# meuleman/epilogos

Measured on AMD Instinct MI355X. Metric: Mbins scored/sec (S1, 18-state, 833 biosamples), higher is better.
Workload: dtype u8

## Files before the change

### epilogos_amd/_abi.py

```python
import ctypes as C
import re
from pathlib import Path

from . import build as _build

EPG_OK = 0
ERR_NAMES = {-1: "EPG_ERR_INVALID_ARG", -2: "EPG_ERR_UNSUPPORTED", -3: "EPG_ERR_HIP", -4: "EPG_ERR_WORKSPACE"}

HEADER = Path(__file__).resolve().parents[1] / "include" / "epilogos_amd.h"


class EpilogosHipError(RuntimeError):
    def __init__(self, code, msg):
        super().__init__("%s (%d): %s" % (ERR_NAMES.get(code, "EPG_ERR"), code, msg))
        self.code = code


_p = C.c_void_p
_i64 = C.c_int64
_i32 = C.c_int32
_u64 = C.c_uint64

PROTOTYPES = {
    "epg_version": (C.c_int, []),
    "epg_last_error": (C.c_char_p, []),
    "epg_device_cus": (C.c_int, []),
    "epg_bin_hist": (C.c_int, [_p, _i64, _i32, _i64, _i32, _p, _p, _p]),
    "epg_bin_hist_s2": (C.c_int, [_p, _i64, _i32, _i64, _i32, _p, _p, _p, _p]),
    "epg_bin_hist_parts": (C.c_int, [_i32, _p, _p, _p, _p, _i32, _p, _p, _p]),
    "epg_hist_s1": (C.c_int, [_p, _i64, _i32, _i64, _i32, _p, _p]),
    "epg_hist_s2": (C.c_int, [_p, _i64, _i32, _i64, _i32, _p, _p, _i64, _p]),
    "epg_hist_s2_from_binhist": (C.c_int, [_p, _i64, _i32, _p, _p]),
    "epg_hist_s2_from_binhist_pair": (C.c_int, [_p, _p, _i64, _i32, _p, _p]),
    "epg_combine_score_s1": (C.c_int, [_p, _i32, _p, _i64, _i32, _i32, _p, _p, _p, _p, _i64, _p]),
    "epg_hist_s3": (C.c_int, [_p, _i64, _i32, _i64, _i32, _p, _p, _i64, _p]),
    "epg_normalise_i64": (C.c_int, [_p, _i64, _p, _p, _i64, _p]),
    "epg_normalise_i32": (C.c_int, [_p, _i64, _p, _p, _i64, _p]),
    "epg_ws_bytes": (_i64, [_i32, _i64, _i32, _i32]),
    "epg_score_s1": (C.c_int, [_p, _i64, _i32, _i64, _i32, _p, _p, _p, _p, _i64, _p]),
    "epg_score_s1_from_binhist": (C.c_int, [_p, _i64, _i32, _i32, _p, _p, _p, _p, _i64, _p]),
    "epg_score_s1_from_binhist_table": (C.c_int, [_p, _i64, _i32, _i32, _p, _p, _p, _p, _p]),
    "epg_pair_scores_s1_from_binhist": (C.c_int, [_p, _p, _p, _p, _i64, _i32, _i32, _i32, _i32, _i32, _p, _p, _p, _p, _p, _p, _p, _p, _p]),
    "epg_pair_scores_s1_parts": (C.c_int, [_i32, _p, _p, _p, _p, _p, _i32, _i32, _i32, _i32, _i32, _p, _p, _p, _p, _p, _p, _p, _p, _p, _i32, _p]),
    "epg_score_s2": (C.c_int, [_p, _i64, _i32, _i64, _i32, _i64, _p, _p, _p, _p, _i64, _p]),
    "epg_score_s2_from_binhist": (C.c_int, [_p, _i64, _i32, _i32, _i64, _p, _p, _p, _p, _i64, _p]),
    "epg_score_s3": (C.c_int, [_p, _i64, _i32, _i64, _i32, _p, _p, _p, _p, _i64, _p]),
    "epg_pair_finish": (C.c_int, [_p, _p, _i64, _i32, _p, _p, _p]),
    "epg_pair_metrics": (C.c_int, [_p, _i64, _i32, _i32, _p, _p, _p]),
    "epg_quiescent": (C.c_int, [_p, _i32, _i64, _p, _i32, _i64, _i64, _i32, _p, _p]),
    "epg_null_hist": (C.c_int, [_p, _i32, _i64, _p, _i32, _i64, _i64, _i32, _i32, _i32, _u64, _i64, _p, _p, _p]),
    "epg_quiescent_from_binhist": (C.c_int, [_p, _p, _i64, _i32, _i32, _i32, _i32, _p, _p]),
    "epg_null_hist_from_binhist": (C.c_int, [_p, _p, _i64, _i32, _i32, _i32, _i32, _u64, _i64, _p, _p, _p]),
    "epg_null_hist_from_binhist_parts": (C.c_int, [_i32, _p, _p, _p, _i32, _i32, _i32, _i32, _u64, _p, _p, _p, _p]),
    "epg_pair_count_null_parts": (C.c_int, [_i32, _p, _p, _p, _i32, _i32, _p, _p, _i32, _p, _p, _p, _u64, _p, _p, _p, _p]),
    "epg_simsearch_ws_bytes": (_i64, [_i64, _i32, _i32, _i32]),
    "epg_simsearch": (C.c_int, [_p, _i64, _i32, _i32, _p, _i32, _p, _i32, _u64, _p, _i64, _p, _p, _p, _p]),
    "epg_simsearch_reduce": (C.c_int, [_p, _i64, _i32, _i32, _p, _p, _p]),
    "epg_simsearch_slices": (C.c_int, [_p, _i64, _i32, _i32, _i32, _p, _i32, _p, _p]),
    "epg_test_force": (C.c_int, [_i32, _i32]),
}

_lib = None


def header_symbols():
    txt = re.sub(r"/\*.*?\*/", "", HEADER.read_text(), flags=re.S)
    return sorted(set(re.findall(r"\b(epg_[a-z0-9_]+)\s*\(", txt)))


def lib_path():
    import os
    p = os.environ.get("EPILOGOS_HIP_LIB")
    return Path(p) if p else _build.LIB_PATH


def _header_abi_version():
    m = re.search(r"^#define\s+EPG_ABI_VERSION\s+(\d+)", HEADER.read_text(), flags=re.M)
    if m is None:
        raise RuntimeError("EPG_ABI_VERSION not found in %s" % HEADER)
    return int(m.group(1))


ABI_VERSION = _header_abi_version()


def load():
    global _lib
    if _lib is not None:
        return _lib
    import torch
    path = lib_path()
    if not path.exists():
        raise EpilogosHipError(-3, "%s is missing: build it with `python -m epilogos_amd.build` "
                                   "(there is no CPU fallback)" % path)
    lib = C.CDLL(str(path))
    for name, (res, args) in PROTOTYPES.items():
        fn = getattr(lib, name)
        fn.restype = res
        fn.argtypes = args
    if lib.epg_version() != ABI_VERSION:
        raise EpilogosHipError(-3, "%s has ABI version %d, this package speaks %d: rebuild it with `python -m epilogos_amd.build`"
                               % (path, lib.epg_version(), ABI_VERSION))
    _lib = lib
    return lib


def check(rc):
    if rc < 0:
        raise EpilogosHipError(rc, load().epg_last_error().decode(errors="replace"))
    return rc


def call(name, *args):
    return check(getattr(load(), name)(*args))
```

### epilogos_amd/build.py

```python
import os
import shutil
import subprocess
from pathlib import Path

PKG = Path(__file__).resolve().parent
ROOT = PKG.parent
CSRC = PKG / "csrc"
LIB_DIR = PKG / "_lib"
LIB_PATH = LIB_DIR / "libepilogos_hip.so"
SOURCES = ["epg_abi.hip", "epg_s1.hip", "epg_s2.hip", "epg_s3.hip", "epg_s3_transpose.hip", "epg_s3_gemm.hip", "epg_s3_lanes.hip", "epg_null.hip", "epg_wide.hip", "epg_simsearch.hip",
           "epg_simsearch_prep.hip"]
HEADERS = [CSRC / "epg_common.h", CSRC / "epg_count.h", ROOT / "include" / "epilogos_amd.h"]
ARCH = "gfx950"


def _hipcc():
    exe = shutil.which("hipcc") or "/opt/rocm/bin/hipcc"
    if not os.path.exists(exe):
        raise RuntimeError("hipcc not found: cannot build libepilogos_hip.so")
    return exe


def is_stale():
    if not LIB_PATH.exists():
        return True
    t = LIB_PATH.stat().st_mtime
    deps = [CSRC / s for s in SOURCES] + HEADERS
    return any(d.stat().st_mtime > t for d in deps)


IO_LIB_PATH = LIB_DIR / "libepilogos_io.so"
IO_SOURCE = CSRC / "epg_io.cpp"
IO_HEADER = ROOT / "include" / "epilogos_io.h"


def io_is_stale():
    if not IO_LIB_PATH.exists():
        return True
    t = IO_LIB_PATH.stat().st_mtime
    return any(f.stat().st_mtime > t for f in (IO_SOURCE, IO_HEADER, CSRC / "epg_deflate.h", CSRC / "epg_inflate.h", CSRC / "epg_crc32.h"))


def build_io_library(force=False, verbose=False):
    if not force and not io_is_stale():
        return IO_LIB_PATH
    LIB_DIR.mkdir(parents=True, exist_ok=True)
    cxx = shutil.which("g++") or shutil.which("c++")
    if cxx is None:
        raise RuntimeError("g++ not found: cannot build libepilogos_io.so")
    tmp = LIB_DIR / (IO_LIB_PATH.name + ".tmp.%d" % os.getpid())
    cmd = [cxx, "-O3", "-std=c++17", "-fPIC", "-shared", "-pthread", "-I" + str(ROOT / "include"), str(IO_SOURCE),
           "-lz", "-o", str(tmp)]
    if verbose:
        print(" ".join(cmd), flush=True)
    res = subprocess.run(cmd, capture_output=True, text=True)
    if res.returncode != 0:
        raise RuntimeError("g++ failed:\n" + res.stdout + res.stderr)
    os.replace(tmp, IO_LIB_PATH)
    return IO_LIB_PATH


OBJ_DIR = LIB_DIR / "obj"


def _compile_one(src, obj, extra_flags, verbose):
    cmd = [_hipcc(), "--offload-arch=" + ARCH, "-O3", "-std=c++17", "-fPIC", "-c",
           "-I" + str(ROOT / "include"), "-I" + str(CSRC), *extra_flags, str(src), "-o", str(obj)]
    if verbose:
        print(" ".join(cmd), flush=True)
    res = subprocess.run(cmd, capture_output=True, text=True)
    if res.returncode != 0:
        raise RuntimeError("hipcc failed on %s:\n%s%s" % (src.name, res.stdout, res.stderr))


def build_library(force=False, verbose=False, extra_flags=()):
    if os.environ.get("EPILOGOS_BUILD_EXPERIMENTS") == "1":
        extra_flags = tuple(extra_flags) + ("-DEPILOGOS_BUILD_EXPERIMENTS",)
    if not force and not is_stale():
        return LIB_PATH
    from concurrent.futures import ThreadPoolExecutor
    OBJ_DIR.mkdir(parents=True, exist_ok=True)
    flag_tag = OBJ_DIR / "flags.txt"
    flags_now = " ".join(extra_flags)
    same_flags = flag_tag.exists() and flag_tag.read_text() == flags_now
    hdr_t = max(h.stat().st_mtime for h in HEADERS)
    todo, objs = [], []
    for s in SOURCES:
        src, obj = CSRC / s, OBJ_DIR / (s + ".o")
        objs.append(obj)
        if force or not same_flags or not obj.exists() or obj.stat().st_mtime < max(src.stat().st_mtime, hdr_t):
            todo.append((src, obj))
    jobs = max(1, min(len(todo), int(os.environ.get("EPILOGOS_BUILD_JOBS", os.cpu_count() or 4))))
    if todo:
        with ThreadPoolExecutor(max_workers=jobs) as pool:
            for f in [pool.submit(_compile_one, src, obj, extra_flags, verbose) for src, obj in todo]:
                f.result()
        flag_tag.write_text(flags_now)
    tmp = LIB_DIR / (LIB_PATH.name + ".tmp.%d" % os.getpid())
    cmd = [_hipcc(), "--offload-arch=" + ARCH, "-fPIC", "-shared", *[str(o) for o in objs], "-o", str(tmp)]
    if verbose:
        print(" ".join(cmd), flush=True)
    res = subprocess.run(cmd, capture_output=True, text=True)
    if res.returncode != 0:
        raise RuntimeError("hipcc link failed:\n" + res.stdout + res.stderr)
    os.replace(tmp, LIB_PATH)
    return LIB_PATH


if __name__ == "__main__":
    print(build_library(force=True, verbose=True))
    print(build_io_library(force=True, verbose=True))
```

### epilogos_amd/csrc/epg_s1.hip

```cpp
#include "epg_count.h"

#include <stdlib.h>
#include <string.h>

namespace epg {

typedef unsigned short k1_v2u16 __attribute__((ext_vector_type(2)));

constexpr int K1P_LD = 17;

template <int SC, bool FULL, bool PAIRS, typename Loop>
__device__ __forceinline__ void bin_hist_body(int Sout_, u64* __restrict__ counts, int nmax, u64* __restrict__ counts2, Loop&& loop) {
    constexpr int S = SC;
    constexpr int ND = (S + 1) / 2;
    const int Sout = FULL ? S : Sout_;
    const int ROWB = 2 * Sout;
    __shared__ u64 s_cnt[S + 1];
    __shared__ __attribute__((aligned(16))) char s_stage[4][32 * 2 * S];
    constexpr int PG = (S + 2) / 3, PSP = 3 * PG, PROLES = PG * (PG + 1) / 2, PSLICE = PROLES <= 64 ? 64 / PROLES : 1;
    static_assert(!PAIRS || (FULL && PROLES <= 64), "the pair counts need a compile-time row width and at most 64 block roles");
    __shared__ u32 s_pair[PAIRS ? 4 * PSP * K1P_LD : 1];
    __shared__ u64 s_c2[PAIRS ? S * S : 1];
    const int lane = threadIdx.x & 63, wave = threadIdx.x >> 6;
    const int j = lane & 3, b = lane >> 2;
    if (threadIdx.x <= S) s_cnt[threadIdx.x] = 0;
    if (PAIRS) {
        for (int e = threadIdx.x; e < S * S; e += 256) s_c2[e] = 0;
        for (int e = threadIdx.x; e < 4 * PSP * K1P_LD; e += 256) s_pair[e] = 0;
    }
    __syncthreads();
    u16* H = nullptr;
    int pgi = -1, pgj = 0, pkq = 0;
    u64 pacc[PAIRS ? 9 : 1], prs[PAIRS ? 3 : 1];
    if (PAIRS) {
        const int role = lane < PROLES * PSLICE ? lane / PSLICE : -1;
        pkq = lane % PSLICE;
        if (role >= 0) {
            int t = role, i = 0;
            while (t >= PG - i) { t -= PG - i; ++i; }
            pgi = i; pgj = i + t;
        }
#pragma unroll
        for (int c = 0; c < 9; ++c) pacc[c] = 0;
#pragma unroll
        for (int c = 0; c < 3; ++c) prs[c] = 0;
    }
    auto pair_counts = [&](const char* stage, int rows) {
        u32* sp = s_pair + wave * PSP * K1P_LD;
        const u16* raw = reinterpret_cast<const u16*>(stage);
        __builtin_amdgcn_wave_barrier();
        for (int e = lane; e < S * 16; e += 64) {
            const int i = e >> 4, k = e & 15;
            const u32 lo = 2 * k < rows ? raw[(2 * k) * S + i] : 0u, hi = 2 * k + 1 < rows ? raw[(2 * k + 1) * S + i] : 0u;
            sp[i * K1P_LD + k] = lo | (hi << 16);
        }
        __builtin_amdgcn_wave_barrier();
        if (pgi >= 0) {
            const u32* pi = sp + 3 * pgi * K1P_LD;
            const u32* pj = sp + 3 * pgj * K1P_LD;
            u32 part[9] = {0, 0, 0, 0, 0, 0, 0, 0, 0}, ps[3] = {0, 0, 0};
            const bool diag = pgi == pgj;
            for (int k = pkq; k < 16; k += PSLICE) {
                const u32 av[3] = {pi[k], pi[K1P_LD + k], pi[2 * K1P_LD + k]};
                const u32 bv[3] = {pj[k], pj[K1P_LD + k], pj[2 * K1P_LD + k]};
#pragma unroll
                for (int t = 0; t < 3; ++t)
#pragma unroll
                    for (int u = 0; u < 3; ++u)
                        part[3 * t + u] = __builtin_amdgcn_udot2(__builtin_bit_cast(k1_v2u16, av[t]), __builtin_bit_cast(k1_v2u16, bv[u]), part[3 * t + u], false);
                if (diag) {
#pragma unroll
                    for (int t = 0; t < 3; ++t)
                        ps[t] = __builtin_amdgcn_udot2(__builtin_bit_cast(k1_v2u16, av[t]), __builtin_bit_cast(k1_v2u16, 0x00010001u), ps[t], false);
                }
            }
#pragma unroll
            for (int c = 0; c < 9; ++c) pacc[c] += part[c];
#pragma unroll
            for (int c = 0; c < 3; ++c) prs[c] += ps[c];
        }
        __builtin_amdgcn_wave_barrier();
    };

    u32 accp[ND];
#pragma unroll
    for (int m = 0; m < ND; ++m) accp[m] = 0;
    const int flush_every = 65535 / nmax > 1 ? 65535 / nmax - 1 : 1;
    int since = 0;
    auto flush = [&]() {
        if (j == 0) {
#pragma unroll
            for (int m = 0; m < ND; ++m) {
                const u32 lo = accp[m] & 0xffffu, hi = accp[m] >> 16;
                if (lo) atomicAdd(&s_cnt[2 * m], (u64)lo);
                if (hi) atomicAdd(&s_cnt[2 * m + 1], (u64)hi);
            }
        }
#pragma unroll
        for (int m = 0; m < ND; ++m) accp[m] = 0;
        since = 0;
    };

    auto enter = [&](u16* Hpart) { H = Hpart; };
    auto epilogue = [&](int half, long row, bool valid, u32 (&cnt)[S]) {
        u32 d[ND];
        pack_reduce<S>(cnt, d);
        if (counts) {
#pragma unroll
            for (int m = 0; m < ND; ++m) accp[m] += valid ? d[m] : 0u;
            if (++since >= flush_every) flush();
        }
        if (H) {
            char* srow = &s_stage[wave][(half * 16 + b) * ROWB];
            if constexpr (FULL && (S & 1) == 0) {
#pragma unroll
                for (int k = 0; k < (ND + 3) / 4; ++k) {
                    const u32 v = sel4(d[4 * k], 4 * k + 1 < ND ? d[4 * k + 1] : 0u, 4 * k + 2 < ND ? d[4 * k + 2] : 0u,
                                       4 * k + 3 < ND ? d[4 * k + 3] : 0u, j);
                    if (4 * k + j < ND) *reinterpret_cast<u32*>(srow + 4 * (4 * k + j)) = v;
                }
            } else {
#pragma unroll
                for (int k = 0; k < (S + 3) / 4; ++k) {
                    const u32 v = (j & 2) ? (2 * k + 1 < ND ? d[2 * k + 1] : 0u) : d[2 * k];
                    const u32 c = (j & 1) ? v >> 16 : v & 0xffffu;
                    if (4 * k + j < Sout) *reinterpret_cast<u16*>(srow + 2 * (4 * k + j)) = (u16)c;
                }
            }
        }
    };
    auto finish = [&](long st, long row0, int rows) {
        if (H) store_staged(s_stage[wave], reinterpret_cast<char*>(H) + row0 * ROWB, rows * ROWB, lane);
        if constexpr (PAIRS) pair_counts(s_stage[wave], rows);
    };
    loop(enter, epilogue, finish);

    if (counts) {
        flush();
        __syncthreads();
        if ((int)threadIdx.x < Sout && s_cnt[threadIdx.x]) atomicAdd(&counts[threadIdx.x], s_cnt[threadIdx.x]);
    }
    if constexpr (PAIRS) {
        if (pgi >= 0) {
            const bool diag = pgi == pgj;
#pragma unroll
            for (int t = 0; t < 3; ++t)
#pragma unroll
                for (int u = 0; u < 3; ++u) {
                    const int i = 3 * pgi + t, jj = 3 * pgj + u;
                    u64 v = pacc[3 * t + u];
                    if (diag && t == u) v -= prs[t];
                    if (i >= S || jj >= S || !v) continue;
                    atomicAdd(&s_c2[i * S + jj], v);
                    if (!diag) atomicAdd(&s_c2[jj * S + i], v);
                }
        }
        __syncthreads();
        for (int e = threadIdx.x; e < S * S; e += 256)
            if (s_c2[e]) atomicAdd(&counts2[e], s_c2[e]);
    }
}

template <int SC, int NG, bool FULL>
__global__ __launch_bounds__(256) void k_bin_hist(const char* __restrict__ X, long R, int N, long ldx, int Sout_,
                                                   u16* __restrict__ H, u64* __restrict__ counts) {
    bin_hist_body<SC, FULL, false>(Sout_, counts, N, nullptr, [&](auto&& enter, auto&& epilogue, auto&& finish) {
        enter(H);
        tile_loop<SC, NG>(X, R, N, ldx, epilogue, finish);
    });
}

template <int SC, int NG>
__global__ __launch_bounds__(256) void k_bin_hist_s2(const char* __restrict__ X, long R, int N, long ldx, u16* __restrict__ H,
                                                      u64* __restrict__ counts, u64* __restrict__ counts2) {
    bin_hist_body<SC, true, true>(SC, counts, N, counts2, [&](auto&& enter, auto&& epilogue, auto&& finish) {
        enter(H);
        tile_loop<SC, NG>(X, R, N, ldx, epilogue, finish);
    });
}

template <int SC, int NG, bool FULL>
__global__ __launch_bounds__(256) void k_bin_hist_parts(const KhParts pt, int Sout_, u64* __restrict__ counts, int nmax) {
    bin_hist_body<SC, FULL, false>(Sout_, counts, nmax, nullptr, [&](auto&& enter, auto&& epilogue, auto&& finish) {
        tile_loop_parts<SC, NG>(pt, [&](int part) { enter(pt.h[part]); }, epilogue, finish);
    });
}

__global__ __launch_bounds__(256) void k_bin_hist_safe(const char* __restrict__ X, long row_begin, long row_end, int N,
                                                        long ldx, int S, u16* __restrict__ H, u64* __restrict__ counts, int mask = 31) {
    __shared__ u32 s_h[4][128];
    const int lane = threadIdx.x & 63, wave = threadIdx.x >> 6;
    for (long row = row_begin + (long)blockIdx.x * 4 + wave; row < row_end; row += (long)gridDim.x * 4) {
        for (int s = lane; s < S; s += 64) s_h[wave][s] = 0;
        __builtin_amdgcn_wave_barrier();
        const char* rp = X + row * ldx;
        for (int n = lane; n < N; n += 64) {
            const int v = (unsigned char)rp[n] & mask;
            if (v < S) atomicAdd(&s_h[wave][v], 1u);
        }
        __builtin_amdgcn_wave_barrier();
        for (int s = lane; s < S; s += 64) {
            const u32 c = s_h[wave][s];
            if (H) H[row * S + s] = (u16)c;
            if (counts && c) atomicAdd(&counts[s], (u64)c);
        }
        __builtin_amdgcn_wave_barrier();
    }
}

__global__ void k_s1_table(const float* __restrict__ q, int N, int S, double* __restrict__ T64, float* __restrict__ T32) {
    const long e = (long)blockIdx.x * blockDim.x + threadIdx.x;
    if (e >= (long)(N + 1) * S) return;
    const int c = (int)(e / S), s = (int)(e % S);
    const double p = (double)c / (double)N;
    const double v = kl_term(p, (double)q[s]);
    T64[e] = v;
    T32[e] = (float)v;
}

template <int S, int NG, typename OT>
__global__ __launch_bounds__(256) void k_score_s1(const char* __restrict__ X, long R, int N, long ldx,
                                                   const OT* __restrict__ T, OT* __restrict__ out) {
    constexpr int ND = (S + 1) / 2;
    constexpr int ROWB = S * (int)sizeof(OT);
    __shared__ __attribute__((aligned(16))) char s_stage[4][32 * ROWB];
    const int lane = threadIdx.x & 63, wave = threadIdx.x >> 6;
    const int j = lane & 3, b = lane >> 2;
    auto epilogue = [&](int half, long row, bool valid, u32 (&cnt)[S]) {
        u32 d[ND];
        pack_reduce<S>(cnt, d);
        OT* srow = reinterpret_cast<OT*>(&s_stage[wave][(half * 16 + b) * ROWB]);
#pragma unroll
        for (int k = 0; k < (S + 3) / 4; ++k) {
            const u32 v = (j & 2) ? (2 * k + 1 < ND ? d[2 * k + 1] : 0u) : d[2 * k];
            const u32 c = (j & 1) ? v >> 16 : v & 0xffffu;
            const int s = 4 * k + j;
            if (s < S) srow[s] = (c && valid) ? T[(long)c * S + s] : (OT)0;
        }
    };
    auto finish = [&](long st, long row0, int rows) {
        store_staged_nt(s_stage[wave], reinterpret_cast<char*>(out) + row0 * ROWB, rows * ROWB, lane);
    };
    tile_loop<S, NG>(X, R, N, ldx, epilogue, finish);
}

template <typename OT, bool LDS_T>
__global__ __launch_bounds__(LDS_T ? 1024 : 256) void k_score_s1_from_hist(const u16* __restrict__ H, long total, int S,
                                                                             const OT* __restrict__ Tg, int nent, OT* __restrict__ out,
                                                                             u64* __restrict__ zero_counts, int rev) {
    extern __shared__ __attribute__((aligned(16))) char smem_t[];
    if (zero_counts && blockIdx.x == 0 && (int)threadIdx.x < S) zero_counts[threadIdx.x] = 0;
    const OT* T = Tg;
    if (LDS_T) {
        OT* Ts = reinterpret_cast<OT*>(smem_t);
        for (int e = threadIdx.x; e < nent; e += blockDim.x) Ts[e] = Tg[e];
        __syncthreads();
        T = Ts;
    }
    const u32 cmax = (u32)(nent / S - 1);
    const long nquads = total >> 2;
    const long stride = (long)gridDim.x * blockDim.x;
    long qd = (long)blockIdx.x * blockDim.x + threadIdx.x;
    const long qtop = nquads - 1, qsgn = rev ? -1 : 1, qoff = rev ? qtop : 0;
    for (; qd + 3 * stride < nquads; qd += 4 * stride) {
        uint2 h[4];
#pragma unroll
        for (int u = 0; u < 4; ++u) h[u] = *reinterpret_cast<const uint2*>(H + 4 * (qoff + qsgn * (qd + u * stride)));
#pragma unroll
        for (int u = 0; u < 4; ++u) {
            const long e0 = 4 * (qoff + qsgn * (qd + u * stride));
            int s = (int)(e0 % S);
            const u32 c[4] = {h[u].x & 0xffffu, h[u].x >> 16, h[u].y & 0xffffu, h[u].y >> 16};
            OT v[4];
#pragma unroll
            for (int k = 0; k < 4; ++k) {
                v[k] = c[k] - 1u < cmax ? T[(long)c[k] * S + s] : (OT)0;
                s = s + 1 == S ? 0 : s + 1;
            }
            if constexpr (sizeof(OT) == 4) {
                typedef float v4f_nt __attribute__((ext_vector_type(4)));
                const v4f_nt vv = {(float)v[0], (float)v[1], (float)v[2], (float)v[3]};
                __builtin_nontemporal_store(vv, reinterpret_cast<v4f_nt*>(out + e0));
            } else {
                typedef double v2d_nt __attribute__((ext_vector_type(2)));
                const v2d_nt lo = {(double)v[0], (double)v[1]}, hi = {(double)v[2], (double)v[3]};
                __builtin_nontemporal_store(lo, reinterpret_cast<v2d_nt*>(out + e0));
                __builtin_nontemporal_store(hi, reinterpret_cast<v2d_nt*>(out + e0 + 2));
            }
        }
    }
    for (; qd < nquads; qd += stride) {
        const long e0 = 4 * (qoff + qsgn * qd);
        int s = (int)(e0 % S);
        for (int k = 0; k < 4; ++k) {
            const u32 c = H[e0 + k];
            out[e0 + k] = c - 1u < cmax ? T[(long)c * S + s] : (OT)0;
            s = s + 1 == S ? 0 : s + 1;
        }
    }
    if (blockIdx.x == 0 && threadIdx.x < (total & 3)) {
        const long e = (nquads << 2) + threadIdx.x;
        const u32 c = H[e];
        out[e] = c - 1u < cmax ? T[(long)c * S + (int)(e % S)] : (OT)0;
    }
}

template <typename IT>
__global__ __launch_bounds__(256) void k_sum_int(const IT* __restrict__ C, long n, long long* __restrict__ total) {
    long long acc = 0;
    for (long i = (long)blockIdx.x * blockDim.x + threadIdx.x; i < n; i += (long)gridDim.x * blockDim.x) acc += (long long)C[i];
    for (int off = 32; off > 0; off >>= 1) acc += __shfl_down(acc, off);
    __shared__ long long s_part[4];
    if ((threadIdx.x & 63) == 0) s_part[threadIdx.x >> 6] = acc;
    __syncthreads();
    if (threadIdx.x == 0) {
        const long long t = s_part[0] + s_part[1] + s_part[2] + s_part[3];
        if (t) atomicAdd(reinterpret_cast<u64*>(total), (u64)t);
    }
}

template <typename IT>
__global__ __launch_bounds__(256) void k_normalise(const IT* __restrict__ C, long n, const long long* __restrict__ total,
                                                    float* __restrict__ q) {
    const double tot = (double)(*total);
    for (long i = (long)blockIdx.x * blockDim.x + threadIdx.x; i < n; i += (long)gridDim.x * blockDim.x)
        q[i] = (float)((double)C[i] / tot);
}

template <typename IT>
__global__ __launch_bounds__(256) void k_normalise_small(const IT* __restrict__ C, int n, float* __restrict__ q) {
    __shared__ long long s_part[4];
    long long acc = 0;
    for (int i = threadIdx.x; i < n; i += 256) acc += (long long)C[i];
    for (int off = 32; off > 0; off >>= 1) acc += __shfl_down(acc, off);
    if ((threadIdx.x & 63) == 0) s_part[threadIdx.x >> 6] = acc;
    __syncthreads();
    const double tot = (double)(s_part[0] + s_part[1] + s_part[2] + s_part[3]);
    for (int i = threadIdx.x; i < n; i += 256) q[i] = (float)((double)C[i] / tot);
}

static int blocks_per_cu() { return g_force[FORCE_K1_BLOCKS_PER_CU] > 0 ? g_force[FORCE_K1_BLOCKS_PER_CU] : 2; }
static int grid_for_tiles(long R) {
    const long nsuper = (R + 31) >> 5;
    long blocks = (nsuper + 3) / 4;
    const long cap = (long)num_cus() * blocks_per_cu();
    if (blocks > cap) {
        const long iters = (nsuper + cap * 4 - 1) / (cap * 4);
        blocks = (nsuper + iters * 4 - 1) / (iters * 4);
    }
    if (blocks < 1) blocks = 1;
    return (int)blocks;
}

template <typename F>
static void with_count_core(int S, int ng, F&& f) {
    if (S == 15 || S == 18 || S == 25)
        with_constant<25, 15, 18>(S, [&](auto sc) {
            with_constant<0, 1, 2, 3, 4, 5, 6, 7, 8>(ng, [&](auto NG) { f(sc, NG, std::true_type{}); });
        });
    else
        with_constant<31, 15, 18, 25>(S < 15 ? 15 : S < 18 ? 18 : S < 25 ? 25 : 31,
                                      [&](auto sc) { f(sc, std::integral_constant<int, 0>{}, std::false_type{}); });
}

static long fast_rows(long R, int N, long ldx) {
    const long chunks = (N + 15) / 16;
    const long over = 16 * chunks - ldx;
    if (over <= 0) return R;
    const long unsafe = (over + ldx - 1) / ldx;
    return R > unsafe ? R - unsafe : 0;
}

extern "C" int epg_bin_hist(const int8_t* X8, int64_t R, int32_t N, int64_t ldx, int32_t S, uint16_t* H, int64_t* counts, void* stream) {
    hipStream_t st = (hipStream_t)stream;
    if (R < 0 || N < 1 || ldx < N || S < 1) return fail(EPG_ERR_INVALID_ARG, "bin_hist: bad shape R=%lld N=%d ldx=%lld S=%d", (long long)R, N, (long long)ldx, S);
    if (S > 127) return fail(EPG_ERR_UNSUPPORTED, "bin_hist: S=%d > 127 (states are int8)", S);
    if (N > 65535) return fail(EPG_ERR_UNSUPPORTED, "bin_hist: N=%d > 65535 (uint16 per-bin counts)", N);
    if (R == 0) return EPG_OK;
    if (!X8) return fail(EPG_ERR_INVALID_ARG, "bin_hist: X is NULL");
    if (H && (reinterpret_cast<uintptr_t>(H) & 15)) return fail(EPG_ERR_INVALID_ARG, "bin_hist: H must be 16-byte aligned");
    const char* X = reinterpret_cast<const char*>(X8);
    u64* cnt = reinterpret_cast<u64*>(counts);
    if (S > 31) {
        hipLaunchKernelGGL(k_bin_hist_safe, dim3((unsigned)((R + 3) / 4 < num_cus() * 32L ? (R + 3) / 4 : num_cus() * 32L)), dim3(256), 0, st, X, 0L,
                           (long)R, N, ldx, S, H, cnt, 255);
        EPG_LAUNCH_CHECK("k_bin_hist_safe");
        return EPG_OK;
    }
    const long Rf = fast_rows(R, N, ldx);
    if (Rf > 0) {
        with_count_core(S, (N + 127) / 128, [&](auto SC, auto NG, auto MODEL) {
            hipLaunchKernelGGL((k_bin_hist<SC, NG, MODEL && (SC & 1) == 0>), dim3(grid_for_tiles(Rf)), dim3(256), 0, st, X, Rf, N, ldx, S, H, cnt);
        });
        EPG_LAUNCH_CHECK("k_bin_hist");
    }
    if (Rf < R) {
        hipLaunchKernelGGL(k_bin_hist_safe, dim3((unsigned)((R - Rf + 3) / 4 < 1024 ? (R - Rf + 3) / 4 : 1024)), dim3(256), 0, st, X, Rf, (long)R, N, ldx, S, H, cnt);
        EPG_LAUNCH_CHECK("k_bin_hist_safe");
    }
    return EPG_OK;
}

extern "C" int epg_bin_hist_s2(const int8_t* X8, int64_t R, int32_t N, int64_t ldx, int32_t S, uint16_t* H, int64_t* counts, int64_t* counts2,
                               void* stream) {
    hipStream_t st = (hipStream_t)stream;
    if (!H || !counts2) return fail(EPG_ERR_INVALID_ARG, "bin_hist_s2: H and counts2 are required");
    const bool fused = (S == 15 || S == 18 || S == 25) && R > 0 && N >= 1 && N <= 1024 && ldx >= N && X8 &&
                       !(reinterpret_cast<uintptr_t>(H) & 15) && fast_rows(R, N, ldx) == R;
    if (!fused) {
        int rc = epg_bin_hist(X8, R, N, ldx, S, H, counts, stream);
        if (rc) return rc;
        return epg_hist_s2_from_binhist(H, R, S, counts2, stream);
    }
    const char* X = reinterpret_cast<const char*>(X8);
    u64* c1 = reinterpret_cast<u64*>(counts);
    u64* c2 = reinterpret_cast<u64*>(counts2);
    with_constant<25, 18, 15>(S, [&](auto SC) {
        with_constant<8, 1, 2, 3, 4, 5, 6, 7>((N + 127) / 128, [&](auto NG) {
            hipLaunchKernelGGL((k_bin_hist_s2<decltype(SC)::value, NG>), dim3(grid_for_tiles(R)), dim3(256), 0, st, X, R, N, ldx, H, c1, c2);
        });
    });
    EPG_LAUNCH_CHECK("k_bin_hist_s2");
    return EPG_OK;
}

extern "C" int epg_bin_hist_parts(int32_t nparts, const int8_t* const* X, const int64_t* R, const int32_t* N, const int64_t* ldx, int32_t S,
                                  uint16_t* const* H, int64_t* counts, void* stream) {
    hipStream_t st = (hipStream_t)stream;
    if (nparts < 0 || (nparts && (!X || !R || !N || !ldx))) return fail(EPG_ERR_INVALID_ARG, "bin_hist_parts: NULL argument array");
    if (S < 1 || S > 127) return fail(EPG_ERR_UNSUPPORTED, "bin_hist_parts: S=%d outside 1..127", S);
    for (int p = 0; p < nparts; ++p) {
        if (R[p] < 0 || (R[p] && (N[p] < 1 || ldx[p] < N[p]))) return fail(EPG_ERR_INVALID_ARG, "bin_hist_parts: bad shape of part %d", p);
        if (R[p] && N[p] > 65535) return fail(EPG_ERR_UNSUPPORTED, "bin_hist_parts: N=%d > 65535 (uint16 per-bin counts)", N[p]);
        if (R[p] && !X[p]) return fail(EPG_ERR_INVALID_ARG, "bin_hist_parts: X of part %d is NULL", p);
        if (H && H[p] && (reinterpret_cast<uintptr_t>(H[p]) & 15)) return fail(EPG_ERR_INVALID_ARG, "bin_hist_parts: H of part %d must be 16-byte aligned", p);
    }
    if (S > 31) {
        for (int p = 0; p < nparts; ++p) {
            const int rc = epg_bin_hist(X[p], R[p], N[p], ldx[p], S, H ? H[p] : nullptr, counts, stream);
            if (rc) return rc;
        }
        return EPG_OK;
    }
    u64* cnt = reinterpret_cast<u64*>(counts);
    auto cls = [](int n) { const int ng = (n + 127) / 128; return ng <= 8 ? ng : 0; };
    bool seen[9] = {false, false, false, false, false, false, false, false, false};
    for (int p = 0; p < nparts; ++p)
        if (R[p]) seen[cls(N[p])] = true;
    for (int c = 0; c <= 8; ++c) {
        if (!seen[c]) continue;
        for (int p0 = 0; p0 < nparts;) {
            KhParts pt;
            memset(&pt, 0, sizeof(pt));
            long supers = 0;
            int nmax = 1, p = p0;
            for (; p < nparts && pt.n < KH_MAXP; ++p) {
                if (!R[p] || cls(N[p]) != c) continue;
                const long Rf = fast_rows(R[p], N[p], ldx[p]);
                if (Rf < R[p]) {
                    hipLaunchKernelGGL(k_bin_hist_safe, dim3((unsigned)((R[p] - Rf + 3) / 4 < 1024 ? (R[p] - Rf + 3) / 4 : 1024)), dim3(256), 0, st,
                                       reinterpret_cast<const char*>(X[p]), Rf, (long)R[p], N[p], (long)ldx[p], S, H ? H[p] : nullptr, cnt);
                    EPG_LAUNCH_CHECK("k_bin_hist_safe");
                }
                if (Rf == 0) continue;
                const int k = pt.n++;
                pt.x[k] = reinterpret_cast<const char*>(X[p]);
                pt.h[k] = H ? H[p] : nullptr;
                pt.rows[k] = Rf;
                pt.ldx[k] = ldx[p];
                pt.n_cols[k] = N[p];
                pt.st0[k] = supers;
                supers += (Rf + 31) / 32;
                if (N[p] > nmax) nmax = N[p];
            }
            pt.st0[pt.n] = supers;
            p0 = p;
            if (pt.n == 0) break;
            with_count_core(S, c, [&](auto SC, auto NG, auto) {
                hipLaunchKernelGGL((k_bin_hist_parts<SC, NG, (NG > 0 && (SC & 1) == 0)>), dim3(grid_for_tiles(supers * 32)), dim3(256), 0, st, pt, S,
                                   cnt, nmax);
            });
            EPG_LAUNCH_CHECK("k_bin_hist_parts");
        }
    }
    return EPG_OK;
}

static int64_t s1_table_bytes(int N, int S) { return align_up((int64_t)(N + 1) * S * 8, 256) + align_up((int64_t)(N + 1) * S * 4, 256); }

int64_t s1_ws_bytes(int64_t R, int N, int S) {
    return s1_table_bytes(N, S) + 256 + align_up(R * S * 2, 256);
}

static int build_s1_table(const float* q, int N, int S, void* ws, double** T64, float** T32, hipStream_t st) {
    *T64 = reinterpret_cast<double*>(ws);
    *T32 = reinterpret_cast<float*>(reinterpret_cast<char*>(ws) + align_up((int64_t)(N + 1) * S * 8, 256));
    const long n = (long)(N + 1) * S;
    hipLaunchKernelGGL(k_s1_table, dim3((int)((n + 255) / 256)), dim3(256), 0, st, q, N, S, *T64, *T32);
    EPG_LAUNCH_CHECK("k_s1_table");
    return EPG_OK;
}
static int check_score_from_hist_args(const uint16_t* H, const double* out64, const float* out32) {
    if ((reinterpret_cast<uintptr_t>(H) & 7) != 0) return fail(EPG_ERR_INVALID_ARG, "score_s1_from_binhist: H must be 8-byte aligned");
    if ((out32 && (reinterpret_cast<uintptr_t>(out32) & 15)) || (out64 && (reinterpret_cast<uintptr_t>(out64) & 15)))
        return fail(EPG_ERR_INVALID_ARG, "score_s1_from_binhist: outputs must be 16-byte aligned");
    return EPG_OK;
}

template <typename OT>
static int launch_score_s1_from_hist_t(const uint16_t* H, long total, int32_t S, const OT* T, int nent, OT* out, u64* zero_counts, hipStream_t st) {
    const size_t tbytes = (size_t)nent * sizeof(OT);
    const int rev = 1;
    if (tbytes <= 150 * 1024) {
        const int per_cu = tbytes <= 75 * 1024 ? 2 : 1;
        long nb = (total / 4 + 4095) / 4096;
        if (nb > (long)num_cus() * per_cu) nb = (long)num_cus() * per_cu;
        if (nb < 1) nb = 1;
        auto kern = k_score_s1_from_hist<OT, true>;
        static DynLds lds_attr;
        EPG_HIP(ensure_dyn_lds(lds_attr, reinterpret_cast<const void*>(kern), 150 * 1024));
        hipLaunchKernelGGL(kern, dim3((int)nb), dim3(1024), tbytes, st, H, total, S, T, nent, out, zero_counts, rev);
    } else {
        long nb = (total / 4 + 1023) / 1024;
        if (nb > num_cus() * 8L) nb = num_cus() * 8L;
        if (nb < 1) nb = 1;
        hipLaunchKernelGGL((k_score_s1_from_hist<OT, false>), dim3((int)nb), dim3(256), 0, st, H, total, S, T, nent, out, zero_counts, rev);
    }
    EPG_LAUNCH_CHECK("k_score_s1_from_hist");
    return EPG_OK;
}

static int launch_score_s1_from_hist(const uint16_t* H, int64_t R, int32_t N, int32_t S, const double* T64, const float* T32,
                                     double* out64, float* out32, hipStream_t st, u64* zero_counts = nullptr) {
    const long total = (long)R * S;
    const int nent = (N + 1) * S;
    int rc = EPG_OK;
    if (out32) rc = launch_score_s1_from_hist_t<float>(H, total, S, T32, nent, out32, zero_counts, st);
    if (!rc && out64) rc = launch_score_s1_from_hist_t<double>(H, total, S, T64, nent, out64, out32 ? nullptr : zero_counts, st);
    return rc;
}


extern "C" int epg_score_s1_from_binhist(const uint16_t* H, int64_t R, int32_t N, int32_t S, const float* q, double* out64, float* out32,
                                         void* ws, int64_t ws_bytes, void* stream) {
    hipStream_t st = (hipStream_t)stream;
    if (R < 0 || N < 1 || S < 1) return fail(EPG_ERR_INVALID_ARG, "score_s1: bad shape");
    if (R == 0) return EPG_OK;
    if (!H || !q || !ws) return fail(EPG_ERR_INVALID_ARG, "score_s1_from_binhist: NULL argument");
    if (ws_bytes < s1_table_bytes(N, S)) return fail(EPG_ERR_WORKSPACE, "score_s1: workspace %lld < %lld bytes", (long long)ws_bytes, (long long)s1_table_bytes(N, S));
    int rc = check_score_from_hist_args(H, out64, out32);
    if (rc) return rc;
    double* T64; float* T32;
    rc = build_s1_table(q, N, S, ws, &T64, &T32, st);
    if (rc) return rc;
    return launch_score_s1_from_hist(H, R, N, S, T64, T32, out64, out32, st);
}

extern "C" int epg_score_s1_from_binhist_table(const uint16_t* H, int64_t R, int32_t N, int32_t S, const double* T64, const float* T32,
                                               double* out64, float* out32, void* stream) {
    if (R < 0 || N < 1 || S < 1) return fail(EPG_ERR_INVALID_ARG, "score_s1: bad shape");
    if (R == 0) return EPG_OK;
    if (!H || (out64 && !T64) || (out32 && !T32)) return fail(EPG_ERR_INVALID_ARG, "score_s1_from_binhist_table: NULL argument");
    if ((T64 && (reinterpret_cast<uintptr_t>(T64) & 7)) || (T32 && (reinterpret_cast<uintptr_t>(T32) & 3)))
        return fail(EPG_ERR_INVALID_ARG, "score_s1_from_binhist_table: misaligned table");
    int rc = check_score_from_hist_args(H, out64, out32);
    if (rc) return rc;
    return launch_score_s1_from_hist(H, R, N, S, T64, T32, out64, out32, (hipStream_t)stream);
}

__global__ __launch_bounds__(256) void k_s1_combine(const u64* __restrict__ counts, int N, int S, float* __restrict__ q,
                                                     double* __restrict__ T64, float* __restrict__ T32) {
    __shared__ long long s_c[128];
    __shared__ double s_q[128];
    const int t = threadIdx.x;
    if (t < S) s_c[t] = (long long)counts[t];
    __syncthreads();
    if (t < S) {
        long long tot = 0;
        for (int s = 0; s < S; ++s) tot += s_c[s];
        const float qf = (float)((double)s_c[t] / (double)tot);
        if (blockIdx.x == 0) q[t] = qf;
        s_q[t] = (double)qf;
    }
    __syncthreads();
    const int e = blockIdx.x * 256 + t;
    if (e < (N + 1) * S) {
        const int c = e / S, s = e - c * S;
        const double v = kl_term((double)c / (double)N, s_q[s]);
        T64[e] = v;
        T32[e] = (float)v;
    }
}

extern "C" int epg_combine_score_s1(int64_t* counts, int32_t rezero, const uint16_t* H, int64_t R, int32_t N, int32_t S, float* q,
                                    double* out64, float* out32, void* ws, int64_t ws_bytes, void* stream) {
    hipStream_t st = (hipStream_t)stream;
    if (R < 0 || N < 1 || S < 1) return fail(EPG_ERR_INVALID_ARG, "combine_score_s1: bad shape R=%lld N=%d S=%d", (long long)R, N, S);
    if (S > 127) return fail(EPG_ERR_UNSUPPORTED, "combine_score_s1: S=%d > 127 (states are int8)", S);
    if (!counts || !q || !ws || (R > 0 && !H)) return fail(EPG_ERR_INVALID_ARG, "combine_score_s1: NULL argument");
    if (ws_bytes < s1_table_bytes(N, S)) return fail(EPG_ERR_WORKSPACE, "combine_score_s1: workspace %lld < %lld bytes", (long long)ws_bytes, (long long)s1_table_bytes(N, S));
    int rc = check_score_from_hist_args(H, out64, out32);
    if (rc) return rc;
    double* T64 = reinterpret_cast<double*>(ws);
    float* T32 = reinterpret_cast<float*>(reinterpret_cast<char*>(ws) + align_up((int64_t)(N + 1) * S * 8, 256));
    const long nent = (long)(N + 1) * S;
    hipLaunchKernelGGL(k_s1_combine, dim3((unsigned)((nent + 255) / 256)), dim3(256), 0, st, reinterpret_cast<const u64*>(counts), N, S, q, T64, T32);
    EPG_LAUNCH_CHECK("k_s1_combine");
    if (R == 0 || (!out32 && !out64)) {
        if (rezero) EPG_HIP(hipMemsetAsync(counts, 0, (size_t)S * 8, st));
        return EPG_OK;
    }
    return launch_score_s1_from_hist(H, R, N, S, T64, T32, out64, out32, st, rezero ? reinterpret_cast<u64*>(counts) : nullptr);
}

extern "C" int epg_hist_s1(const int8_t* X, int64_t R, int32_t N, int64_t ldx, int32_t S, int64_t* counts, void* stream) {
    if (!counts) return fail(EPG_ERR_INVALID_ARG, "hist_s1: counts is NULL");
    return epg_bin_hist(X, R, N, ldx, S, nullptr, counts, stream);
}

extern "C" int epg_score_s1(const int8_t* X8, int64_t R, int32_t N, int64_t ldx, int32_t S, const float* q, double* out64, float* out32,
                            void* ws, int64_t ws_bytes, void* stream) {
    hipStream_t st = (hipStream_t)stream;
    if (R < 0 || N < 1 || ldx < N || S < 1) return fail(EPG_ERR_INVALID_ARG, "score_s1: bad shape");
    if (S > 127) return fail(EPG_ERR_UNSUPPORTED, "score_s1: S=%d > 127 (states are int8)", S);
    if (R == 0) return EPG_OK;
    if (!X8 || !q || !ws) return fail(EPG_ERR_INVALID_ARG, "score_s1: NULL argument");
    if ((out32 && (reinterpret_cast<uintptr_t>(out32) & 15)) || (out64 && (reinterpret_cast<uintptr_t>(out64) & 15)))
        return fail(EPG_ERR_INVALID_ARG, "score_s1: outputs must be 16-byte aligned");
    const long Rf = fast_rows(R, N, ldx);
    const bool fused = S == 18 && Rf == R;
    if (!fused) {
        if (ws_bytes < s1_ws_bytes(R, N, S)) return fail(EPG_ERR_WORKSPACE, "score_s1: workspace %lld < %lld bytes", (long long)ws_bytes, (long long)s1_ws_bytes(R, N, S));
        u16* H = reinterpret_cast<u16*>(reinterpret_cast<char*>(ws) + s1_table_bytes(N, S));
        int rc = epg_bin_hist(X8, R, N, ldx, S, H, nullptr, stream);
        if (rc) return rc;
        return epg_score_s1_from_binhist(H, R, N, S, q, out64, out32, ws, s1_table_bytes(N, S), stream);
    }
    if (ws_bytes < s1_table_bytes(N, S)) return fail(EPG_ERR_WORKSPACE, "score_s1: workspace %lld < %lld bytes", (long long)ws_bytes, (long long)s1_table_bytes(N, S));
    double* T64; float* T32;
    int rc = build_s1_table(q, N, S, ws, &T64, &T32, st);
    if (rc) return rc;
    const char* X = reinterpret_cast<const char*>(X8);
    with_constant<0, 1, 2, 3, 4, 5, 6, 7, 8>((N + 127) / 128, [&](auto NG) {
        if (out32) hipLaunchKernelGGL((k_score_s1<18, NG, float>), dim3(grid_for_tiles(R)), dim3(256), 0, st, X, R, N, ldx, T32, out32);
        if (out64) hipLaunchKernelGGL((k_score_s1<18, NG, double>), dim3(grid_for_tiles(R)), dim3(256), 0, st, X, R, N, ldx, T64, out64);
    });
    EPG_LAUNCH_CHECK("k_score_s1");
    return EPG_OK;
}

template <typename IT>
static int normalise_impl(const IT* C, int64_t n, float* q, void* ws, int64_t ws_bytes, hipStream_t st) {
    if (n < 1 || !C || !q || !ws) return fail(EPG_ERR_INVALID_ARG, "normalise: bad argument");
    if (ws_bytes < 8) return fail(EPG_ERR_WORKSPACE, "normalise: workspace needs 8 bytes");
    if (n <= 4096) {
        hipLaunchKernelGGL((k_normalise_small<IT>), dim3(1), dim3(256), 0, st, C, (int)n, q);
        EPG_LAUNCH_CHECK("k_normalise_small");
        return EPG_OK;
    }
    long long* total = reinterpret_cast<long long*>(ws);
    EPG_HIP(hipMemsetAsync(total, 0, 8, st));
    long blocks = (n + 255) / 256;
    if (blocks > num_cus() * 8L) blocks = num_cus() * 8L;
    hipLaunchKernelGGL((k_sum_int<IT>), dim3((int)blocks), dim3(256), 0, st, C, (long)n, total);
    hipLaunchKernelGGL((k_normalise<IT>), dim3((int)blocks), dim3(256), 0, st, C, (long)n, total, q);
    EPG_LAUNCH_CHECK("k_normalise");
    return EPG_OK;
}

extern "C" int epg_normalise_i64(const int64_t* C, int64_t n, float* q, void* ws, int64_t ws_bytes, void* stream) {
    return normalise_impl<long long>(reinterpret_cast<const long long*>(C), n, q, ws, ws_bytes, (hipStream_t)stream);
}
extern "C" int epg_normalise_i32(const int32_t* C, int64_t n, float* q, void* ws, int64_t ws_bytes, void* stream) {
    return normalise_impl<int>(C, n, q, ws, ws_bytes, (hipStream_t)stream);
}

}
```

### epilogos_amd/engine.py

```python
import ctypes as C

import numpy as np
import torch

from . import _abi
from ._abi import EpilogosHipError

ROW_ALIGN = 16


def require_gpu():
    if not torch.cuda.is_available():
        raise EpilogosHipError(-3, "no HIP device visible to torch: the epilogos_amd engine has no CPU fallback")
    _abi.load()


def _ptr(t):
    return C.c_void_p(t.data_ptr()) if t is not None else None


def _stream():
    return C.c_void_p(torch.cuda.current_stream().cuda_stream)


def padded_width(N):
    return (N + ROW_ALIGN - 1) // ROW_ALIGN * ROW_ALIGN


def alloc_states(R, N, device="cuda"):
    return torch.empty((R, padded_width(N)), dtype=torch.int8, device=device)


PLACE_MIN_BYTES = 1 << 30
PLACE_BLOCK = 4 << 30
PLACE_SEARCH_AT = 2
PLACE_TRIES = 8
PLACE_BUDGET_MS = 50.0
PLACE_DEEP_AT = 4
PLACE_DEEP_TRIES = 24
PLACE_DEEP_WALL_MS = 5000.0
PLACE_GAP = 0.03
PLACE_SURE = 1.10
PLACE_WIN = 0.01
_placement = {}


def _storage_users(t):
    f = getattr(torch._C, "_storage_Use_Count", None)
    if f is None:
        return None
    return int(f(t.untyped_storage()._cdata)) - 1


def _probe_slices(R, rows=1 << 20):
    m = min(rows, R // 3) // 32 * 32
    if m <= 0:
        return [(0, R)]
    return [(0, m), ((R - m) // 2 // 32 * 32, (R - m) // 2 // 32 * 32 + m), ((R - m) // 32 * 32, (R - m) // 32 * 32 + m)]


def _probe_ms(X, N, S, Hflat, counts, slices, reps=2):
    ev = [torch.cuda.Event(enable_timing=True) for _ in range(2)]
    H = None if Hflat is None else Hflat[:X.shape[0] * S * 2].view(torch.int16).view(X.shape[0], S)
    for k in range(reps + 1):
        if k == 1:
            ev[0].record()
        for lo, hi in slices:
            bin_hist(X[lo:hi], N, S, counts=counts, H=None if H is None else H[lo:hi], want_hist=H is not None)
    ev[1].record()
    ev[1].synchronize()
    return ev[0].elapsed_time(ev[1]) / reps


def place_decide(ratios, excluded=(), gap=PLACE_GAP, sure=PLACE_SURE):
    live = [i for i in range(len(ratios)) if i not in set(excluded)]
    if not live:
        return None, "none"
    order = sorted(live, key=lambda i: ratios[i])
    best = order[0]
    if ratios[best] <= sure:
        return best, "sure"
    allo = sorted(range(len(ratios)), key=lambda i: ratios[i])
    steps = [(ratios[allo[k + 1]] / ratios[allo[k]] - 1.0, k) for k in range(len(allo) - 1)]
    if steps:
        step, k = max(steps)
        if step >= gap:
            lower = [i for i in allo[:k + 1] if i not in set(excluded)]
            if lower:
                return lower[0], "two-levels"
    return best, "one-level"


def placement_enabled():
    import os
    if os.environ.get("EPILOGOS_PLACEMENT", "1") == "0" or getattr(torch._C, "_storage_Use_Count", None) is None:
        return False
    try:
        lws = int(os.environ.get("LOCAL_WORLD_SIZE", "1"))
    except ValueError:
        lws = 1
    return lws <= max(torch.cuda.device_count(), 1)


def _order_after_last_user(st):
    prev, cur = st.get("stream"), torch.cuda.current_stream()
    if prev is not None and prev != cur:
        ev = torch.cuda.Event()
        ev.record(prev)
        cur.wait_event(ev)
    st["stream"] = cur


def alloc_hist(X, N, S):
    import os
    R = X.shape[0]
    dev = X.device
    hbytes = R * S * 2
    plain = lambda: torch.empty((R, S), dtype=torch.int16, device=dev)
    if X.numel() < PLACE_MIN_BYTES or not placement_enabled():
        return plain()
    st = _placement.get(dev.index)
    stor = X.untyped_storage()
    key = (stor.data_ptr(), stor.nbytes())
    view = lambda home: home[:hbytes].view(torch.int16).view(R, S)
    eager = os.environ.get("EPILOGOS_PLACEMENT_EAGER") == "1"
    if st is not None and st["home"] is not None and st["home"].numel() >= hbytes:
        users = _storage_users(st["home"])
        if users is None or users > 1:
            st["report"]["plain_while_home_in_use"] = st["report"].get("plain_while_home_in_use", 0) + 1
            return plain()
        if st["key"] == key:
            st["report"]["reuses"] = st["report"].get("reuses", 0) + 1
            _order_after_last_user(st)
            return view(st["home"])
        counts = zeros_counts(S, device=dev)
        slices = _probe_slices(R)
        r = _probe_ms(X, N, S, st["home"], counts, slices) / _probe_ms(X, N, S, None, counts, slices)
        if r <= PLACE_SURE:
            st["key"] = key
            st["report"].update(revalidated=st["report"].get("revalidated", 0) + 1, ratio=round(r, 3))
            _order_after_last_user(st)
            return view(st["home"])
        st = None
        _placement.pop(dev.index, None)
    if st is None or st["key"] != key:
        st = _placement[dev.index] = {"key": key, "home": None, "report": {"jobs_seen": 0, "tier": "none yet"}, "stream": None, "seen": 0, "tier": 0}
    st["seen"] += 1
    st["report"]["jobs_seen"] = st["seen"]
    want = 0
    if st["tier"] < 1 and (eager or st["seen"] >= PLACE_SEARCH_AT):
        want = 1
    elif st["tier"] == 1 and (eager or st["seen"] >= PLACE_DEEP_AT):
        want = 2
    if not want:
        return plain()
    deep = want == 2
    home, h_plain, report = _place_search(X, N, S, int(os.environ.get("EPILOGOS_PLACEMENT_TRIES", PLACE_DEEP_TRIES if deep else PLACE_TRIES)),
                                          3 * PLACE_BUDGET_MS if deep else PLACE_BUDGET_MS, PLACE_DEEP_WALL_MS if deep else 10 * PLACE_BUDGET_MS,
                                          stop_at_slow_alloc=not deep)
    report.update(tier="deep" if deep else "quick", jobs_seen=st["seen"], reuses=0)
    if deep and "quick" not in report:
        report["quick"] = {k: st["report"].get(k) for k in ("decision", "ratios", "blocks_tried", "search_ms")}
    if home is None and report["picked"] == 0 and report["decision"].startswith("plain allocation kept (sure"):
        want = 2
    st.update(home=home, report=report, stream=torch.cuda.current_stream(), tier=want)
    if home is None and eager and want == 1:
        return alloc_hist(X, N, S)
    return view(home) if home is not None else h_plain


PLACE_SLOW_ALLOC_MS = 20.0


def _place_search(X, N, S, tries, budget_ms, wall_ms, stop_at_slow_alloc=False):
    import time
    R = X.shape[0]
    dev = X.device
    hbytes = R * S * 2
    t_start = time.perf_counter()
    counts = zeros_counts(S, device=dev)
    slices = _probe_slices(R)
    whole = [(0, R)]
    spent = [0.0]

    def probe(cand, where, reps=2):
        ms = _probe_ms(X, N, S, cand, counts, where, reps=reps)
        spent[0] += ms * (reps + 1)
        return ms

    base = probe(None, slices)
    block = max(PLACE_BLOCK, (hbytes + 4095) // 4096 * 4096)
    h_plain = torch.empty((R, S), dtype=torch.int16, device=dev)
    cands, ratios = [h_plain.view(torch.int8).view(-1)], []
    t0 = probe(cands[0], slices)
    base = min(base, probe(None, slices))
    ratios.append(t0 / base)
    whole_ms, excluded, alloc_ms = {}, [], []

    def walk_on():
        k = len(cands) - 1
        if k >= tries or spent[0] >= budget_ms or (time.perf_counter() - t_start) * 1e3 >= wall_ms:
            return False
        if stop_at_slow_alloc and alloc_ms and alloc_ms[-1] > PLACE_SLOW_ALLOC_MS:
            return False
        free, _total = torch.cuda.mem_get_info(dev)
        if free < block + 16 * hbytes + (8 << 30):
            return False
        t0 = time.perf_counter()
        try:
            cands.append(torch.empty(block, dtype=torch.int8, device=dev))
        except RuntimeError:
            return False
        torch.cuda.synchronize(dev)
        alloc_ms.append((time.perf_counter() - t0) * 1e3)
        ratios.append(probe(cands[-1], slices) / base)
        return True

    pick, verdict = place_decide(ratios, excluded)
    while True:
        while verdict not in ("sure", "two-levels") and walk_on():
            pick, verdict = place_decide(ratios, excluded)
        if pick in (None, 0):
            break
        if slices == whole:
            whole_ms = {0: ratios[0] * base, pick: ratios[pick] * base}
        else:
            if 0 not in whole_ms:
                whole_ms[0] = probe(cands[0], whole, reps=1)
            whole_ms[pick] = probe(cands[pick], whole, reps=1)
        if whole_ms[pick] < whole_ms[0] * (1.0 - PLACE_WIN):
            break
        excluded.append(pick)
        if len(excluded) >= 3 or spent[0] >= 2 * budget_ms:
            pick = 0
            break
        pick, verdict = place_decide(ratios, excluded)
        verdict += " (after %d pick(s) that lost over the whole matrix)" % len(excluded)
    if pick is None or pick in excluded:
        pick = 0
    good = pick != 0
    report = {"probe": "k_bin_hist over 3 x %d bins of the matrix: with the H store into a candidate / counts only; candidate 0 is the plain "
                       "allocation, the others heads of %d GiB blocks allocated one after the other" % (slices[0][1] - slices[0][0], block >> 30),
              "decision": verdict if good else "plain allocation kept (%s)" % verdict, "good": good, "picked": pick, "ratio": round(ratios[pick], 3),
              "ratios": [round(r, 3) for r in ratios], "whole_matrix_ms": {str(i): round(v, 4) for i, v in whole_ms.items()},
              "lost_over_the_whole_matrix": excluded, "blocks_tried": len(cands) - 1,
              "walked_GiB": round(sum(c.numel() for c in cands[1:]) / 2**30, 1),
              "block_alloc_ms": [round(a, 1) for a in alloc_ms],
              "rules": {"sure_at_or_under": PLACE_SURE, "two_levels_apart_by": PLACE_GAP, "must_beat_plain_by": PLACE_WIN,
                        "max_blocks": tries, "max_probe_ms": budget_ms, "max_wall_ms": wall_ms},
              "ms_counts_only": round(base, 4), "probe_device_ms": round(spent[0], 2),
              "left_in_torch_cache_GiB": round(sum(c.numel() for i, c in enumerate(cands) if i and i != pick) / 2**30, 1)}
    home = cands[pick] if good else None
    del cands
    report["search_ms"] = round((time.perf_counter() - t_start) * 1e3, 2)
    return home, h_plain, report


def placement_report(device=None):
    idx = torch.cuda.current_device() if device is None else torch.device(device).index
    st = _placement.get(idx)
    return None if st is None else dict(st["report"])


def release_placement():
    _placement.clear()


def states_to_device(x, device="cuda"):
    x = np.ascontiguousarray(x)
    R, N = x.shape
    ldx = padded_width(N)
    host = np.full((R, ldx), -1, dtype=np.int8)
    host[:, :N] = x.astype(np.int8)
    return torch.from_numpy(host).to(device)


def _check_states(X, N):
    if X.dtype != torch.int8 or X.dim() != 2 or not X.is_cuda or X.stride(1) != 1:
        raise ValueError("state matrix must be a 2-D int8 CUDA tensor with unit column stride")
    if N > X.shape[1]:
        raise ValueError("N exceeds the row width")
    return X.shape[0], X.stride(0)


def zeros_counts(n, dtype=torch.int64, device="cuda"):
    return torch.zeros(n, dtype=dtype, device=device)


def bin_hist(X, N, S, want_hist=True, counts=None, want_counts=True, H=None):
    R, ldx = _check_states(X, N)
    if H is None and want_hist:
        H = torch.empty((R, S), dtype=torch.int16, device=X.device)
    if want_counts and counts is None:
        counts = zeros_counts(S, device=X.device)
    _abi.call("epg_bin_hist", _ptr(X), R, N, ldx, S, _ptr(H), _ptr(counts) if want_counts else None, _stream())
    return H, counts


def bin_hist_s2(X, N, S, counts2=None, H=None, counts=None):
    R, ldx = _check_states(X, N)
    if H is None:
        H = torch.empty((R, S), dtype=torch.int16, device=X.device)
    if counts2 is None:
        counts2 = zeros_counts(S * S, device=X.device)
    _abi.call("epg_bin_hist_s2", _ptr(X), R, N, ldx, S, _ptr(H), _ptr(counts), _ptr(counts2), _stream())
    return H, counts2


def _ptr_array(ts):
    return (C.c_void_p * len(ts))(*[t.data_ptr() if t is not None and t.numel() else None for t in ts])


def hist_rows_flat(rows, S, device, dtype=torch.int16):
    starts, at = [], 0
    for r in rows:
        starts.append(at)
        at += (r + 7) // 8 * 8
    return torch.empty((max(at, 1), S), dtype=dtype, device=device), starts


def hist_rows_alloc(rows, S, device):
    flat, starts = hist_rows_flat(rows, S, device)
    return [flat[a:a + r] for a, r in zip(starts, rows)]


def bin_hist_parts(Xs, Ns, S, counts=None, want_hist=True, Hs=None):
    n = len(Xs)
    if n == 0:
        return [], counts
    shapes = [_check_states(X, N) if X.shape[0] else (0, max(N, 1)) for X, N in zip(Xs, Ns)]
    dev = Xs[0].device
    if Hs is None and want_hist:
        Hs = hist_rows_alloc([r for r, _l in shapes], S, dev)
    _abi.call("epg_bin_hist_parts", n, _ptr_array(Xs), (C.c_int64 * n)(*[r for r, _l in shapes]), (C.c_int32 * n)(*[int(N or 1) for N in Ns]),
              (C.c_int64 * n)(*[l for _r, l in shapes]), S, _ptr_array(Hs) if Hs is not None else None, _ptr(counts), _stream())
    return Hs, counts


def null_hist_from_binhist_parts(HAs, HBs, n_cols, S, ga, gb, seed, row0s, stream=None):
    n = len(HAs)
    if n == 0:
        return [], []
    rows = [h.shape[0] for h in HAs]
    dev = HAs[0].device
    OAs, OBs = hist_rows_alloc(rows, S, dev), hist_rows_alloc(rows, S, dev)
    _abi.call("epg_null_hist_from_binhist_parts", n, _ptr_array(HAs), _ptr_array(HBs), (C.c_int64 * n)(*rows), S, n_cols, ga, gb, seed,
              (C.c_int64 * n)(*[int(r) for r in row0s]), _ptr_array(OAs), _ptr_array(OBs),
              _stream() if stream is None else C.c_void_p(stream.cuda_stream))
    return OAs, OBs


def pair_count_null_parts(XAs, XBs, NA, NB, S, seed, row0s, counts=None):
    n = len(XAs)
    sa = [_check_states(X, NA) if X.shape[0] else (0, padded_width(NA)) for X in XAs]
    sb = [_check_states(X, NB) if X.shape[0] else (0, padded_width(NB)) for X in XBs]
    rows = [r for r, _l in sa]
    if rows != [r for r, _l in sb]:
        raise ValueError("paired inputs must have the same number of bins")
    dev = XAs[0].device
    H = hist_rows_alloc(rows + rows, S, dev)
    O = hist_rows_alloc(rows + rows, S, dev)
    _abi.call("epg_pair_count_null_parts", n, _ptr_array(XAs), _ptr_array(XBs), (C.c_int64 * n)(*rows), NA, NB,
              (C.c_int64 * n)(*[l for _r, l in sa]), (C.c_int64 * n)(*[l for _r, l in sb]), S, _ptr_array(H[:n]), _ptr_array(H[n:]),
              _ptr(counts), seed, (C.c_int64 * n)(*[int(r) for r in row0s]), _ptr_array(O[:n]), _ptr_array(O[n:]), _stream())
    return H[:n], H[n:], O[:n], O[n:]


def hist_s2_from_binhist(H, S, counts=None):
    if counts is None:
        counts = zeros_counts(S * S, device=H.device)
    _abi.call("epg_hist_s2_from_binhist", _ptr(H), H.shape[0], S, _ptr(counts), _stream())
    return counts


def hist_s2_from_binhist_pair(HA, HB, S, counts=None):
    if HA.shape != HB.shape:
        raise ValueError("paired histograms must have the same shape")
    if counts is None:
        counts = zeros_counts(S * S, device=HA.device)
    _abi.call("epg_hist_s2_from_binhist_pair", _ptr(HA), _ptr(HB), HA.shape[0], S, _ptr(counts), _stream())
    return counts


def hist_s3_ws_bytes(R, N, S):
    return max(int(_abi.call("epg_ws_bytes", 3, R, N, S)), 256)


def hist_s3(X, N, S, counts=None, use_workspace=True, ws=None):
    R, ldx = _check_states(X, N)
    if counts is None:
        counts = zeros_counts(N * N * S * S, dtype=torch.int32, device=X.device)
    if use_workspace:
        if ws is None:
            ws = torch.empty(hist_s3_ws_bytes(R, N, S), dtype=torch.uint8, device=X.device)
        _abi.call("epg_hist_s3", _ptr(X), R, N, ldx, S, _ptr(counts), _ptr(ws), ws.numel(), _stream())
    else:
        _abi.call("epg_hist_s3", _ptr(X), R, N, ldx, S, _ptr(counts), None, 0, _stream())
    return counts


def normalise(counts, q=None, ws=None):
    if q is None:
        q = torch.empty(counts.numel(), dtype=torch.float32, device=counts.device)
    if ws is None:
        ws = torch.empty(256, dtype=torch.uint8, device=counts.device)
    name = {torch.int64: "epg_normalise_i64", torch.int32: "epg_normalise_i32"}[counts.dtype]
    _abi.call(name, _ptr(counts), counts.numel(), _ptr(q), _ptr(ws), ws.numel(), _stream())
    return q


def _outs(R, S, device, want32, want64, out32=None, out64=None):
    o32 = out32 if out32 is not None else (torch.empty((R, S), dtype=torch.float32, device=device) if want32 else None)
    o64 = out64 if out64 is not None else (torch.empty((R, S), dtype=torch.float64, device=device) if want64 else None)
    return o32, o64


def workspace(saliency, R, N, S, device="cuda"):
    return _ws(saliency, R, N, S, device)


def _ws(saliency, R, N, S, device):
    nbytes = _abi.call("epg_ws_bytes", saliency, R, N, S)
    return torch.empty(max(nbytes, 256), dtype=torch.uint8, device=device)


def score_s1(X, N, S, q, want32=True, want64=False, out32=None, out64=None, ws=None):
    R, ldx = _check_states(X, N)
    o32, o64 = _outs(R, S, X.device, want32, want64, out32, out64)
    if ws is None:
        ws = _ws(1, R, N, S, X.device)
    _abi.call("epg_score_s1", _ptr(X), R, N, ldx, S, _ptr(q), _ptr(o64), _ptr(o32), _ptr(ws), ws.numel(), _stream())
    return o32, o64


def score_s1_from_binhist(H, N, S, q, want32=True, want64=False, out32=None, out64=None, ws=None):
    R = H.shape[0]
    o32, o64 = _outs(R, S, H.device, want32, want64, out32, out64)
    if ws is None:
        ws = _ws(1, 0, N, S, H.device)
    _abi.call("epg_score_s1_from_binhist", _ptr(H), R, N, S, _ptr(q), _ptr(o64), _ptr(o32), _ptr(ws), ws.numel(),
              _stream())
    return o32, o64


def score_s1_from_binhist_table(H, N, S, T64=None, T32=None, out32=None, out64=None):
    R = H.shape[0]
    for T, dt in ((T64, torch.float64), (T32, torch.float32)):
        if T is not None and (T.dtype != dt or T.numel() != (N + 1) * S or not T.is_contiguous()):
            raise ValueError("S1 table must be a contiguous [N + 1, S] tensor of its output's dtype")
    o32, o64 = _outs(R, S, H.device, T32 is not None, T64 is not None, out32, out64)
    _abi.call("epg_score_s1_from_binhist_table", _ptr(H), R, N, S, _ptr(T64), _ptr(T32), _ptr(o64), _ptr(o32), _stream())
    return o32, o64


def combine_score_s1(counts, H, N, S, q=None, want32=True, want64=False, out32=None, out64=None, ws=None, rezero=False):
    R = H.shape[0]
    o32, o64 = _outs(R, S, H.device, want32, want64, out32, out64)
    if q is None:
        q = torch.empty(S, dtype=torch.float32, device=H.device)
    if ws is None:
        ws = _ws(1, 0, N, S, H.device)
    _abi.call("epg_combine_score_s1", _ptr(counts), 1 if rezero else 0, _ptr(H), R, N, S, _ptr(q), _ptr(o64), _ptr(o32),
              _ptr(ws), ws.numel(), _stream())
    return q, o32, o64


def s1_tables(counts, N, S, q=None, ws=None):
    dev = counts.device
    if q is None:
        q = torch.empty(S, dtype=torch.float32, device=dev)
    if ws is None:
        ws = _ws(1, 0, N, S, dev)
    _abi.call("epg_combine_score_s1", _ptr(counts), 0, None, 0, N, S, _ptr(q), None, None, _ptr(ws), ws.numel(), _stream())
    nent = (N + 1) * S
    off = (nent * 8 + 255) // 256 * 256
    return q, ws[:nent * 8].view(torch.float64), ws[off:off + nent * 4].view(torch.float32)


def score_s2(X, N, S, q, perms=None, want32=True, want64=False):
    R, ldx = _check_states(X, N)
    perms = N * (N - 1) if perms is None else perms
    o32, o64 = _outs(R, S, X.device, want32, want64)
    ws = _ws(2, R, N, S, X.device)
    _abi.call("epg_score_s2", _ptr(X), R, N, ldx, S, perms, _ptr(q), _ptr(o64), _ptr(o32), _ptr(ws), ws.numel(),
              _stream())
    return o32, o64


def score_s2_from_binhist(H, N, S, q, perms=None, want32=True, want64=False, out32=None, out64=None, ws=None):
    R = H.shape[0]
    perms = N * (N - 1) if perms is None else perms
    o32, o64 = _outs(R, S, H.device, want32, want64, out32, out64)
    if ws is None:
        ws = _ws(2, 0, N, S, H.device)
    _abi.call("epg_score_s2_from_binhist", _ptr(H), R, N, S, perms, _ptr(q), _ptr(o64), _ptr(o32), _ptr(ws),
              ws.numel(), _stream())
    return o32, o64


def score_s3(X, N, S, q, want32=True, want64=False, ws=None):
    R, ldx = _check_states(X, N)
    o32, o64 = _outs(R, S, X.device, want32, want64)
    if ws is None:
        ws = _ws(3, R, N, S, X.device)
    _abi.call("epg_score_s3", _ptr(X), R, N, ldx, S, _ptr(q), _ptr(o64), _ptr(o32), _ptr(ws), ws.numel(), _stream())
    return o32, o64


def pair_scores_s1_from_binhist(HA, HB, HnA, HnB, S, NA, NB, ga, gb, TA, TB, TnA, TnB):
    R = HA.shape[0]
    dev = HA.device
    delta = torch.empty((R, S), dtype=torch.float32, device=dev)
    null = torch.empty(R, dtype=torch.float32, device=dev)
    dist = torch.empty(R, dtype=torch.float32, device=dev)
    maxdiff = torch.empty(R, dtype=torch.int32, device=dev)
    _abi.call("epg_pair_scores_s1_from_binhist", _ptr(HA), _ptr(HB), _ptr(HnA), _ptr(HnB), R, S, NA, NB, ga, gb, _ptr(TA), _ptr(TB), _ptr(TnA),
              _ptr(TnB), _ptr(delta), _ptr(null), _ptr(dist), _ptr(maxdiff), _stream())
    return delta, null, dist, maxdiff


def pair_scores_s1_parts(parts, S, NA, NB, ga, gb, TA, TB, TnA, TnB, qstate=None):
    n = len(parts)
    if n == 0:
        return []
    dev = parts[0][0].device
    outs = []
    for HA, _HB, _HnA, _HnB in parts:
        R = HA.shape[0]
        outs.append({"delta": torch.empty((R, S), dtype=torch.float32, device=dev), "null": torch.empty(R, dtype=torch.float32, device=dev),
                     "rdist": torch.empty(R, dtype=torch.float32, device=dev), "mdiff": torch.empty(R, dtype=torch.int32, device=dev),
                     "quies": torch.empty(R, dtype=torch.uint8, device=dev) if qstate is not None else None})
    arr = lambda ts: (C.c_void_p * n)(*[t.data_ptr() if t is not None and t.numel() else None for t in ts])
    rows = (C.c_int64 * n)(*[p[0].shape[0] for p in parts])
    _abi.call("epg_pair_scores_s1_parts", n, arr([p[0] for p in parts]), arr([p[1] for p in parts]), arr([p[2] for p in parts]),
              arr([p[3] for p in parts]), rows, S, NA, NB, ga, gb, _ptr(TA), _ptr(TB), _ptr(TnA), _ptr(TnB), arr([o["delta"] for o in outs]),
              arr([o["null"] for o in outs]), arr([o["rdist"] for o in outs]), arr([o["mdiff"] for o in outs]),
              arr([o["quies"] for o in outs]) if qstate is not None else None, -1 if qstate is None else int(qstate), _stream())
    return outs


def pair_finish(a, b, want_dist=True):
    R, S = a.shape
    delta = torch.empty_like(a)
    dist = torch.empty(R, dtype=torch.float32, device=a.device) if want_dist else None
    _abi.call("epg_pair_finish", _ptr(a), _ptr(b), R, S, _ptr(delta), _ptr(dist), _stream())
    return delta, dist


def pair_metrics(delta, roundtrip=True):
    R, S = delta.shape
    dist = torch.empty(R, dtype=torch.float32, device=delta.device)
    maxdiff = torch.empty(R, dtype=torch.int32, device=delta.device)
    _abi.call("epg_pair_metrics", _ptr(delta), R, S, 1 if roundtrip else 0, _ptr(dist), _ptr(maxdiff), _stream())
    return dist, maxdiff


def quiescent(XA, NA, XB, NB, qstate):
    R, ldxa = _check_states(XA, NA)
    R2, ldxb = _check_states(XB, NB)
    if R != R2:
        raise ValueError("paired inputs must have the same number of bins")
    mask = torch.empty(R, dtype=torch.uint8, device=XA.device)
    _abi.call("epg_quiescent", _ptr(XA), NA, ldxa, _ptr(XB), NB, ldxb, R, qstate, _ptr(mask), _stream())
    return mask


def null_hist(XA, NA, XB, NB, S, ga, gb, seed, row0=0):
    R, ldxa = _check_states(XA, NA)
    _, ldxb = _check_states(XB, NB)
    HA = torch.empty((R, S), dtype=torch.int16, device=XA.device)
    HB = torch.empty((R, S), dtype=torch.int16, device=XA.device)
    _abi.call("epg_null_hist", _ptr(XA), NA, ldxa, _ptr(XB), NB, ldxb, R, S, ga, gb, seed, row0, _ptr(HA), _ptr(HB),
              _stream())
    return HA, HB


_hip_rt = None


def _pinned_bytes(nbytes):
    global _hip_rt
    if _hip_rt is None:
        for name in ("libamdhip64.so", "libamdhip64.so.7", "libamdhip64.so.6"):
            try:
                _hip_rt = C.CDLL(name)
                break
            except OSError:
                continue
        if _hip_rt is None:
            _hip_rt = False
    if _hip_rt:
        import weakref
        ptr = C.c_void_p()
        if _hip_rt.hipHostMalloc(C.byref(ptr), C.c_size_t(int(nbytes)), C.c_uint(0)) == 0 and ptr.value:
            base = (C.c_int8 * int(nbytes)).from_address(ptr.value)
            weakref.finalize(base, _hip_rt.hipHostFree, C.c_void_p(ptr.value))
            t = torch.from_numpy(np.frombuffer(base, dtype=np.int8))
            if t.is_pinned():
                return t
            del t
    return torch.empty(int(nbytes), dtype=torch.int8, pin_memory=True)


class PinnedPool:

    def __init__(self, n_buffers=3, in_order=True):
        import threading
        self.cv = threading.Condition()
        self.free = [None] * n_buffers
        self.next = 0
        self.in_order = in_order
        self.aborted = False
        self.weights = {}
        self.target = 0
        self.waiting = set()
        self.closed = False

    def hint(self, weights):
        self.weights = dict(weights)

    def abort(self):
        with self.cv:
            self.aborted = True
            self.cv.notify_all()

    def acquire(self, ticket, nbytes):
        import os, sys, time
        trace = os.environ.get("EPILOGOS_TIMING") == "2"
        t_in = time.perf_counter()
        with self.cv:
            self.waiting.add(ticket)
            first = lambda: not self.weights or self.weights.get(ticket, 0) >= max(self.weights.get(t, 0) for t in self.waiting)
            self.cv.wait_for(lambda: self.aborted or ((not self.in_order or self.next == ticket) and len(self.free) > 0 and first()))
            self.waiting.discard(ticket)
            if self.aborted:
                raise RuntimeError("staging pool aborted")
            buf = self.free.pop()
            self.next += 1
            self.cv.notify_all()
        w = self.weights.get(ticket)
        if w and nbytes:
            self.target = max(self.target, int(nbytes / w * max(self.weights.values()) * 1.05))
        t_got = time.perf_counter()
        grew = 0
        if buf is None or buf.numel() < nbytes:
            buf = None
            buf = _pinned_bytes(max(int(nbytes), self.target, 1 << 20))
            grew = buf.numel()
        if trace:
            print("    [pool] ticket %2d: waited %.2f s for a staging buffer%s  (at %.3f)" % (
                ticket, t_got - t_in, ", page-locked %.2f GB in %.2f s" % (grew / 1e9, time.perf_counter() - t_got) if grew else "",
                time.perf_counter()), file=sys.stderr, flush=True)
        return buf

    def skip(self, ticket):
        if not self.in_order:
            return
        with self.cv:
            self.cv.wait_for(lambda: self.aborted or self.next >= ticket)
            if self.next == ticket:
                self.next += 1
            self.cv.notify_all()

    def release(self, buf):
        with self.cv:
            if self.closed:
                return
            self.free.append(buf)
            self.cv.notify_all()

    def close(self, background=True):
        import threading
        with self.cv:
            self.closed = True
            bufs, self.free = [b for b in self.free if b is not None], []
        if not bufs:
            return

        def work(bufs=bufs):
            while bufs:
                bufs.pop()
        if background:
            threading.Thread(target=work, name="epilogos-staging-close", daemon=True).start()
        else:
            work()


def upload_states(pinned, R, ldx, copy_stream, device="cuda"):
    with torch.cuda.stream(copy_stream):
        X = torch.empty((R, ldx), dtype=torch.int8, device=device)
        if R:
            X.copy_(pinned[:R * ldx].view(R, ldx), non_blocking=True)
        ev = torch.cuda.Event()
        ev.record(copy_stream)
    X.record_stream(torch.cuda.current_stream())
    return X, ev


def quiescent_from_binhist(HA, NA, HB, NB, S, qstate):
    R = HA.shape[0]
    mask = torch.empty(R, dtype=torch.uint8, device=HA.device)
    _abi.call("epg_quiescent_from_binhist", _ptr(HA), _ptr(HB), R, S, NA, NB, qstate, _ptr(mask), _stream())
    return mask


def null_hist_from_binhist(HA, HB, n_cols, S, ga, gb, seed, row0=0, stream=None):
    if HA.shape != HB.shape:
        raise ValueError("paired histograms must have the same shape")
    OA, OB = torch.empty_like(HA), torch.empty_like(HB)
    _abi.call("epg_null_hist_from_binhist", _ptr(HA), _ptr(HB), HA.shape[0], S, n_cols, ga, gb, seed, row0, _ptr(OA), _ptr(OB),
              _stream() if stream is None else C.c_void_p(stream.cuda_stream))
    return OA, OB


def hist_to_numpy(H):
    return H.cpu().numpy().view(np.uint16)
```

Baseline: 5804.

## Pack per-bin S1 histograms as three 10-bit counts per 32-bit word

Adds a packed histogram layout that stores three 10-bit state counts in each uint32 instead of one uint16 per state. It provides packed variants of bin_hist, bin_hist_parts, the table-based S1 scoring and combine_score_s1, including a new scoring kernel that decodes the packed words. The aim is to cut the histogram's memory footprint and the bytes moved between counting and scoring. It only applies when S is a multiple of 3 up to 30 and N is at most 1023, and the engine picks the packed path only when the histogram tensor is int32, so whether the default pipeline uses it is not shown.

```diff
diff --git a/epilogos_amd/_abi.py b/epilogos_amd/_abi.py
--- a/epilogos_amd/_abi.py
+++ b/epilogos_amd/_abi.py
@@ -60,7 +60,20 @@
     "epg_test_force": (C.c_int, [_i32, _i32]),
 }
 
+PRIVATE_HEADER = Path(__file__).resolve().parent / "csrc" / "epg_packed.h"
+PRIVATE_PROTOTYPES = {
+    "epgs_bin_hist_packed": (C.c_int, [_p, _i64, _i32, _i64, _i32, _p, _p, _p]),
+    "epgs_bin_hist_parts_packed": (C.c_int, [_i32, _p, _p, _p, _p, _i32, _p, _p, _p]),
+    "epgs_score_s1_from_packed_table": (C.c_int, [_p, _i64, _i32, _i32, _p, _p, _p, _p, _p]),
+    "epgs_combine_score_s1_packed": (C.c_int, [_p, _i32, _p, _i64, _i32, _i32, _p, _p, _p, _p, _i64, _p]),
+}
+
 _lib = None
+
+
+def private_header_symbols():
+    txt = re.sub(r"/\*.*?\*/", "", PRIVATE_HEADER.read_text(), flags=re.S)
+    return sorted(set(re.findall(r"\b(epgs_[a-z0-9_]+)\s*\(", txt)))
 
 
 def header_symbols():
@@ -94,7 +107,7 @@
         raise EpilogosHipError(-3, "%s is missing: build it with `python -m epilogos_amd.build` "
                                    "(there is no CPU fallback)" % path)
     lib = C.CDLL(str(path))
-    for name, (res, args) in PROTOTYPES.items():
+    for name, (res, args) in list(PROTOTYPES.items()) + list(PRIVATE_PROTOTYPES.items()):
         fn = getattr(lib, name)
         fn.restype = res
         fn.argtypes = args
diff --git a/epilogos_amd/build.py b/epilogos_amd/build.py
--- a/epilogos_amd/build.py
+++ b/epilogos_amd/build.py
@@ -10,7 +10,7 @@
 LIB_PATH = LIB_DIR / "libepilogos_hip.so"
 SOURCES = ["epg_abi.hip", "epg_s1.hip", "epg_s2.hip", "epg_s3.hip", "epg_s3_transpose.hip", "epg_s3_gemm.hip", "epg_s3_lanes.hip", "epg_null.hip", "epg_wide.hip", "epg_simsearch.hip",
            "epg_simsearch_prep.hip"]
-HEADERS = [CSRC / "epg_common.h", CSRC / "epg_count.h", ROOT / "include" / "epilogos_amd.h"]
+HEADERS = [CSRC / "epg_common.h", CSRC / "epg_count.h", CSRC / "epg_packed.h", ROOT / "include" / "epilogos_amd.h"]
 ARCH = "gfx950"
 
 
diff --git a/epilogos_amd/csrc/epg_packed.h b/epilogos_amd/csrc/epg_packed.h
--- /dev/null
+++ b/epilogos_amd/csrc/epg_packed.h
@@ -0,0 +1,21 @@
+#pragma once
+#include <stdint.h>
+
+#ifdef __cplusplus
+extern "C" {
+#endif
+
+int epgs_bin_hist_packed(const int8_t* X, int64_t R, int32_t N, int64_t ldx, int32_t S, uint32_t* P, int64_t* counts, void* stream);
+
+int epgs_bin_hist_parts_packed(int32_t nparts, const int8_t* const* X, const int64_t* R, const int32_t* N, const int64_t* ldx, int32_t S,
+                               uint32_t* const* P, int64_t* counts, void* stream);
+
+int epgs_score_s1_from_packed_table(const uint32_t* P, int64_t R, int32_t N, int32_t S, const double* T64, const float* T32, double* out64,
+                                    float* out32, void* stream);
+
+int epgs_combine_score_s1_packed(int64_t* counts, int32_t rezero, const uint32_t* P, int64_t R, int32_t N, int32_t S, float* q, double* out64,
+                                 float* out32, void* ws, int64_t ws_bytes, void* stream);
+
+#ifdef __cplusplus
+}
+#endif
diff --git a/epilogos_amd/csrc/epg_s1.hip b/epilogos_amd/csrc/epg_s1.hip
--- a/epilogos_amd/csrc/epg_s1.hip
+++ b/epilogos_amd/csrc/epg_s1.hip
@@ -1,4 +1,5 @@
 #include "epg_count.h"
+#include "epg_packed.h"
 
 #include <stdlib.h>
 #include <string.h>
@@ -9,12 +10,15 @@
 
 constexpr int K1P_LD = 17;
 
-template <int SC, bool FULL, bool PAIRS, typename Loop>
+template <int SC, bool FULL, bool PAIRS, bool PACK = false, typename Loop>
 __device__ __forceinline__ void bin_hist_body(int Sout_, u64* __restrict__ counts, int nmax, u64* __restrict__ counts2, Loop&& loop) {
     constexpr int S = SC;
     constexpr int ND = (S + 1) / 2;
+    constexpr int PWC = (S + 2) / 3;
+    static_assert(!(PACK && PAIRS), "the pair counts read uint16 rows");
     const int Sout = FULL ? S : Sout_;
-    const int ROWB = 2 * Sout;
+    const int PW = FULL ? PWC : (Sout + 2) / 3;
+    const int ROWB = PACK ? 4 * PW : 2 * Sout;
     __shared__ u64 s_cnt[S + 1];
     __shared__ __attribute__((aligned(16))) char s_stage[4][32 * 2 * S];
     constexpr int PG = (S + 2) / 3, PSP = 3 * PG, PROLES = PG * (PG + 1) / 2, PSLICE = PROLES <= 64 ? 64 / PROLES : 1;
@@ -112,7 +116,15 @@
         }
         if (H) {
             char* srow = &s_stage[wave][(half * 16 + b) * ROWB];
-            if constexpr (FULL && (S & 1) == 0) {
+            if constexpr (PACK) {
+                auto c = [&](int s) { return s < S && (FULL || s < Sout) ? (d[s >> 1] >> (16 * (s & 1))) & 0xffffu : 0u; };
+                auto p = [&](int k) { return k < PWC ? c(3 * k) | (c(3 * k + 1) << 10) | (c(3 * k + 2) << 20) : 0u; };
+#pragma unroll
+                for (int k = 0; k < (PWC + 3) / 4; ++k) {
+                    const u32 v = sel4(p(4 * k), p(4 * k + 1), p(4 * k + 2), p(4 * k + 3), j);
+                    if (4 * k + j < PW) *reinterpret_cast<u32*>(srow + 4 * (4 * k + j)) = v;
+                }
+            } else if constexpr (FULL && (S & 1) == 0) {
 #pragma unroll
                 for (int k = 0; k < (ND + 3) / 4; ++k) {
                     const u32 v = sel4(d[4 * k], 4 * k + 1 < ND ? d[4 * k + 1] : 0u, 4 * k + 2 < ND ? d[4 * k + 2] : 0u,
@@ -161,10 +173,10 @@
     }
 }
 
-template <int SC, int NG, bool FULL>
+template <int SC, int NG, bool FULL, bool PACK = false>
 __global__ __launch_bounds__(256) void k_bin_hist(const char* __restrict__ X, long R, int N, long ldx, int Sout_,
                                                    u16* __restrict__ H, u64* __restrict__ counts) {
-    bin_hist_body<SC, FULL, false>(Sout_, counts, N, nullptr, [&](auto&& enter, auto&& epilogue, auto&& finish) {
+    bin_hist_body<SC, FULL, false, PACK>(Sout_, counts, N, nullptr, [&](auto&& enter, auto&& epilogue, auto&& finish) {
         enter(H);
         tile_loop<SC, NG>(X, R, N, ldx, epilogue, finish);
     });
@@ -179,15 +191,16 @@
     });
 }
 
-template <int SC, int NG, bool FULL>
+template <int SC, int NG, bool FULL, bool PACK = false>
 __global__ __launch_bounds__(256) void k_bin_hist_parts(const KhParts pt, int Sout_, u64* __restrict__ counts, int nmax) {
-    bin_hist_body<SC, FULL, false>(Sout_, counts, nmax, nullptr, [&](auto&& enter, auto&& epilogue, auto&& finish) {
+    bin_hist_body<SC, FULL, false, PACK>(Sout_, counts, nmax, nullptr, [&](auto&& enter, auto&& epilogue, auto&& finish) {
         tile_loop_parts<SC, NG>(pt, [&](int part) { enter(pt.h[part]); }, epilogue, finish);
     });
 }
 
 __global__ __launch_bounds__(256) void k_bin_hist_safe(const char* __restrict__ X, long row_begin, long row_end, int N,
-                                                        long ldx, int S, u16* __restrict__ H, u64* __restrict__ counts, int mask = 31) {
+                                                        long ldx, int S, u16* __restrict__ H, u64* __restrict__ counts, int mask = 31,
+                                                        int pack = 0) {
     __shared__ u32 s_h[4][128];
     const int lane = threadIdx.x & 63, wave = threadIdx.x >> 6;
     for (long row = row_begin + (long)blockIdx.x * 4 + wave; row < row_end; row += (long)gridDim.x * 4) {
@@ -201,8 +214,17 @@
         __builtin_amdgcn_wave_barrier();
         for (int s = lane; s < S; s += 64) {
             const u32 c = s_h[wave][s];
-            if (H) H[row * S + s] = (u16)c;
+            if (H && !pack) H[row * S + s] = (u16)c;
             if (counts && c) atomicAdd(&counts[s], (u64)c);
+        }
+        if (H && pack) {
+            const int W = (S + 2) / 3;
+            if (lane < W) {
+                u32 v = 0;
+                for (int t = 0; t < 3; ++t)
+                    if (3 * lane + t < S) v |= s_h[wave][3 * lane + t] << (10 * t);
+                reinterpret_cast<u32*>(H)[row * W + lane] = v;
+            }
         }
         __builtin_amdgcn_wave_barrier();
     }
@@ -305,6 +327,98 @@
     }
 }
 
+template <typename OT, bool LDS_T>
+__global__ __launch_bounds__(LDS_T ? 1024 : 256, LDS_T && sizeof(OT) == 4 ? 8 : 4) void k_score_s1_from_packed(const u32* __restrict__ P, long total, int S,
+                                                                               const OT* __restrict__ Tg, int nent, OT* __restrict__ out,
+                                                                               u64* __restrict__ zero_counts, int rev) {
+    extern __shared__ __attribute__((aligned(16))) char smem_t[];
+    if (zero_counts && blockIdx.x == 0 && (int)threadIdx.x < S) zero_counts[threadIdx.x] = 0;
+    const OT* T = Tg;
+    if (LDS_T) {
+        OT* Ts = reinterpret_cast<OT*>(smem_t);
+        for (int e = threadIdx.x; e < nent; e += blockDim.x) Ts[e] = Tg[e];
+        __syncthreads();
+        T = Ts;
+    }
+    const u32 cmax = (u32)(nent / S - 1);
+    const long nquads = total >> 2;
+    const long stride = (long)gridDim.x * blockDim.x;
+    long qd = (long)blockIdx.x * blockDim.x + threadIdx.x;
+    const long qtop = nquads - 1, qsgn = rev ? -1 : 1, qoff = rev ? qtop : 0;
+    const long cstep = 4 * stride;
+    long step_d = cstep / 3;
+    int step_r = (int)(cstep % 3), step_s = (int)(cstep % S);
+    if (rev) {
+        step_d = step_r ? -step_d - 1 : -step_d;
+        step_r = step_r ? 3 - step_r : 0;
+        step_s = step_s ? S - step_s : 0;
+    }
+    const long e_first = qd < nquads ? 4 * (qoff + qsgn * qd) : 0;
+    const u32* p = P + e_first / 3;
+    int r = (int)(e_first % 3), st = (int)(e_first % S);
+    OT* o = out + e_first;
+    const long ostep = qsgn * cstep;
+    auto advance = [&]() {
+        r += step_r;
+        const int carry = r >= 3 ? 1 : 0;
+        p += step_d + carry;
+        r -= 3 * carry;
+        st += step_s;
+        st -= st >= S ? S : 0;
+    };
+    auto load2 = [&](const u32* q) {
+        uint2 v;
+        __builtin_memcpy(&v, q, 8);
+        return v;
+    };
+    auto quad = [&](const uint2& h, int slot, int s, OT* dst) {
+        const u64 z = (u64)(h.x & 0x3fffffffu) | ((u64)(h.y & 0x3fffffffu) << 30);
+        const u64 y = z >> (10 * slot);
+        const u32 lo = (u32)y;
+        const u32 c[4] = {lo & 0x3ffu, (lo >> 10) & 0x3ffu, (lo >> 20) & 0x3ffu, (u32)(y >> 30) & 0x3ffu};
+        OT v[4];
+#pragma unroll
+        for (int k = 0; k < 4; ++k) {
+            v[k] = c[k] - 1u < cmax ? T[(int)c[k] * S + s] : (OT)0;
+            s = s + 1 == S ? 0 : s + 1;
+        }
+        if constexpr (sizeof(OT) == 4) {
+            typedef float v4f_nt __attribute__((ext_vector_type(4)));
+            const v4f_nt vv = {(float)v[0], (float)v[1], (float)v[2], (float)v[3]};
+            __builtin_nontemporal_store(vv, reinterpret_cast<v4f_nt*>(dst));
+        } else {
+            typedef double v2d_nt __attribute__((ext_vector_type(2)));
+            const v2d_nt lo2 = {(double)v[0], (double)v[1]}, hi2 = {(double)v[2], (double)v[3]};
+            __builtin_nontemporal_store(lo2, reinterpret_cast<v2d_nt*>(dst));
+            __builtin_nontemporal_store(hi2, reinterpret_cast<v2d_nt*>(dst + 2));
+        }
+    };
+    for (; qd + 3 * stride < nquads; qd += 4 * stride) {
+        uint2 h[4];
+        int rr[4], ss[4];
+#pragma unroll
+        for (int u = 0; u < 4; ++u) {
+            h[u] = load2(p);
+            rr[u] = r;
+            ss[u] = st;
+            advance();
+        }
+#pragma unroll
+        for (int u = 0; u < 4; ++u) quad(h[u], rr[u], ss[u], o + u * ostep);
+        o += 4 * ostep;
+    }
+    for (; qd < nquads; qd += stride) {
+        quad(load2(p), r, st, o);
+        advance();
+        o += ostep;
+    }
+    if (blockIdx.x == 0 && threadIdx.x < (total & 3)) {
+        const long e = (nquads << 2) + threadIdx.x;
+        const u32 c = (P[e / 3] >> (10 * (int)(e % 3))) & 0x3ffu;
+        out[e] = c - 1u < cmax ? T[(int)c * S + (int)(e % S)] : (OT)0;
+    }
+}
+
 template <typename IT>
 __global__ __launch_bounds__(256) void k_sum_int(const IT* __restrict__ C, long n, long long* __restrict__ total) {
     long long acc = 0;
@@ -371,11 +485,22 @@
     return R > unsafe ? R - unsafe : 0;
 }
 
-extern "C" int epg_bin_hist(const int8_t* X8, int64_t R, int32_t N, int64_t ldx, int32_t S, uint16_t* H, int64_t* counts, void* stream) {
+static int check_packed(const char* who, int N, int S) {
+    if (S > 30 || S % 3) return fail(EPG_ERR_UNSUPPORTED, "%s: S=%d is not a multiple of 3 up to 30 (packed rows)", who, S);
+    if (N > 1023) return fail(EPG_ERR_UNSUPPORTED, "%s: N=%d > 1023 (10-bit per-bin counts)", who, N);
+    return EPG_OK;
+}
+
+static int bin_hist_impl(const int8_t* X8, int64_t R, int32_t N, int64_t ldx, int32_t S, void* Hv, bool pack, int64_t* counts, void* stream) {
     hipStream_t st = (hipStream_t)stream;
+    u16* H = reinterpret_cast<u16*>(Hv);
     if (R < 0 || N < 1 || ldx < N || S < 1) return fail(EPG_ERR_INVALID_ARG, "bin_hist: bad shape R=%lld N=%d ldx=%lld S=%d", (long long)R, N, (long long)ldx, S);
     if (S > 127) return fail(EPG_ERR_UNSUPPORTED, "bin_hist: S=%d > 127 (states are int8)", S);
     if (N > 65535) return fail(EPG_ERR_UNSUPPORTED, "bin_hist: N=%d > 65535 (uint16 per-bin counts)", N);
+    if (pack) {
+        const int rc = check_packed("bin_hist_packed", N, S);
+        if (rc) return rc;
+    }
     if (R == 0) return EPG_OK;
     if (!X8) return fail(EPG_ERR_INVALID_ARG, "bin_hist: X is NULL");
     if (H && (reinterpret_cast<uintptr_t>(H) & 15)) return fail(EPG_ERR_INVALID_ARG, "bin_hist: H must be 16-byte aligned");
@@ -390,15 +515,27 @@
     const long Rf = fast_rows(R, N, ldx);
     if (Rf > 0) {
         with_count_core(S, (N + 127) / 128, [&](auto SC, auto NG, auto MODEL) {
-            hipLaunchKernelGGL((k_bin_hist<SC, NG, MODEL && (SC & 1) == 0>), dim3(grid_for_tiles(Rf)), dim3(256), 0, st, X, Rf, N, ldx, S, H, cnt);
+            if (pack) {
+                if constexpr (!decltype(MODEL)::value || decltype(SC)::value % 3 == 0)
+                    hipLaunchKernelGGL((k_bin_hist<SC, NG, MODEL, true>), dim3(grid_for_tiles(Rf)), dim3(256), 0, st, X, Rf, N, ldx, S, H, cnt);
+            } else hipLaunchKernelGGL((k_bin_hist<SC, NG, MODEL && (SC & 1) == 0>), dim3(grid_for_tiles(Rf)), dim3(256), 0, st, X, Rf, N, ldx, S, H, cnt);
         });
         EPG_LAUNCH_CHECK("k_bin_hist");
     }
     if (Rf < R) {
-        hipLaunchKernelGGL(k_bin_hist_safe, dim3((unsigned)((R - Rf + 3) / 4 < 1024 ? (R - Rf + 3) / 4 : 1024)), dim3(256), 0, st, X, Rf, (long)R, N, ldx, S, H, cnt);
+        hipLaunchKernelGGL(k_bin_hist_safe, dim3((unsigned)((R - Rf + 3) / 4 < 1024 ? (R - Rf + 3) / 4 : 1024)), dim3(256), 0, st, X, Rf, (long)R, N, ldx, S, H, cnt,
+                           31, pack ? 1 : 0);
         EPG_LAUNCH_CHECK("k_bin_hist_safe");
     }
     return EPG_OK;
+}
+
+extern "C" int epg_bin_hist(const int8_t* X, int64_t R, int32_t N, int64_t ldx, int32_t S, uint16_t* H, int64_t* counts, void* stream) {
+    return bin_hist_impl(X, R, N, ldx, S, H, false, counts, stream);
+}
+
+extern "C" int epgs_bin_hist_packed(const int8_t* X, int64_t R, int32_t N, int64_t ldx, int32_t S, uint32_t* P, int64_t* counts, void* stream) {
+    return bin_hist_impl(X, R, N, ldx, S, P, true, counts, stream);
 }
 
 extern "C" int epg_bin_hist_s2(const int8_t* X8, int64_t R, int32_t N, int64_t ldx, int32_t S, uint16_t* H, int64_t* counts, int64_t* counts2,
@@ -424,11 +561,16 @@
     return EPG_OK;
 }
 
-extern "C" int epg_bin_hist_parts(int32_t nparts, const int8_t* const* X, const int64_t* R, const int32_t* N, const int64_t* ldx, int32_t S,
-                                  uint16_t* const* H, int64_t* counts, void* stream) {
+static int bin_hist_parts_impl(int32_t nparts, const int8_t* const* X, const int64_t* R, const int32_t* N, const int64_t* ldx, int32_t S,
+                               void* const* Hv, bool pack, int64_t* counts, void* stream) {
     hipStream_t st = (hipStream_t)stream;
+    u16* const* H = reinterpret_cast<u16* const*>(Hv);
     if (nparts < 0 || (nparts && (!X || !R || !N || !ldx))) return fail(EPG_ERR_INVALID_ARG, "bin_hist_parts: NULL argument array");
     if (S < 1 || S > 127) return fail(EPG_ERR_UNSUPPORTED, "bin_hist_parts: S=%d outside 1..127", S);
+    for (int p = 0; pack && p < nparts; ++p) {
+        const int rc = check_packed("bin_hist_parts_packed", R[p] ? N[p] : 1, S);
+        if (rc) return rc;
+    }
     for (int p = 0; p < nparts; ++p) {
         if (R[p] < 0 || (R[p] && (N[p] < 1 || ldx[p] < N[p]))) return fail(EPG_ERR_INVALID_ARG, "bin_hist_parts: bad shape of part %d", p);
         if (R[p] && N[p] > 65535) return fail(EPG_ERR_UNSUPPORTED, "bin_hist_parts: N=%d > 65535 (uint16 per-bin counts)", N[p]);
@@ -459,7 +601,7 @@
                 const long Rf = fast_rows(R[p], N[p], ldx[p]);
                 if (Rf < R[p]) {
                     hipLaunchKernelGGL(k_bin_hist_safe, dim3((unsigned)((R[p] - Rf + 3) / 4 < 1024 ? (R[p] - Rf + 3) / 4 : 1024)), dim3(256), 0, st,
-                                       reinterpret_cast<const char*>(X[p]), Rf, (long)R[p], N[p], (long)ldx[p], S, H ? H[p] : nullptr, cnt);
+                                       reinterpret_cast<const char*>(X[p]), Rf, (long)R[p], N[p], (long)ldx[p], S, H ? H[p] : nullptr, cnt, 31, pack ? 1 : 0);
                     EPG_LAUNCH_CHECK("k_bin_hist_safe");
                 }
                 if (Rf == 0) continue;
@@ -476,14 +618,27 @@
             pt.st0[pt.n] = supers;
             p0 = p;
             if (pt.n == 0) break;
-            with_count_core(S, c, [&](auto SC, auto NG, auto) {
-                hipLaunchKernelGGL((k_bin_hist_parts<SC, NG, (NG > 0 && (SC & 1) == 0)>), dim3(grid_for_tiles(supers * 32)), dim3(256), 0, st, pt, S,
-                                   cnt, nmax);
+            with_count_core(S, c, [&](auto SC, auto NG, auto MODEL) {
+                if (pack) {
+                    if constexpr (!decltype(MODEL)::value || decltype(SC)::value % 3 == 0)
+                        hipLaunchKernelGGL((k_bin_hist_parts<SC, NG, (NG > 0), true>), dim3(grid_for_tiles(supers * 32)), dim3(256), 0, st, pt, S, cnt, nmax);
+                } else hipLaunchKernelGGL((k_bin_hist_parts<SC, NG, (NG > 0 && (SC & 1) == 0)>), dim3(grid_for_tiles(supers * 32)), dim3(256), 0, st, pt, S,
+                                        cnt, nmax);
             });
             EPG_LAUNCH_CHECK("k_bin_hist_parts");
         }
     }
     return EPG_OK;
+}
+
+extern "C" int epg_bin_hist_parts(int32_t nparts, const int8_t* const* X, const int64_t* R, const int32_t* N, const int64_t* ldx, int32_t S,
+                                  uint16_t* const* H, int64_t* counts, void* stream) {
+    return bin_hist_parts_impl(nparts, X, R, N, ldx, S, reinterpret_cast<void* const*>(H), false, counts, stream);
+}
+
+extern "C" int epgs_bin_hist_parts_packed(int32_t nparts, const int8_t* const* X, const int64_t* R, const int32_t* N, const int64_t* ldx, int32_t S,
+                                          uint32_t* const* P, int64_t* counts, void* stream) {
+    return bin_hist_parts_impl(nparts, X, R, N, ldx, S, reinterpret_cast<void* const*>(P), true, counts, stream);
 }
 
 static int64_t s1_table_bytes(int N, int S) { return align_up((int64_t)(N + 1) * S * 8, 256) + align_up((int64_t)(N + 1) * S * 4, 256); }
@@ -500,43 +655,53 @@
     EPG_LAUNCH_CHECK("k_s1_table");
     return EPG_OK;
 }
-static int check_score_from_hist_args(const uint16_t* H, const double* out64, const float* out32) {
-    if ((reinterpret_cast<uintptr_t>(H) & 7) != 0) return fail(EPG_ERR_INVALID_ARG, "score_s1_from_binhist: H must be 8-byte aligned");
+static int check_score_from_hist_args(const void* H, const double* out64, const float* out32, int h_align = 8) {
+    if ((reinterpret_cast<uintptr_t>(H) & (h_align - 1)) != 0) return fail(EPG_ERR_INVALID_ARG, "score_s1_from_binhist: H must be %d-byte aligned", h_align);
     if ((out32 && (reinterpret_cast<uintptr_t>(out32) & 15)) || (out64 && (reinterpret_cast<uintptr_t>(out64) & 15)))
         return fail(EPG_ERR_INVALID_ARG, "score_s1_from_binhist: outputs must be 16-byte aligned");
     return EPG_OK;
 }
 
-template <typename OT>
-static int launch_score_s1_from_hist_t(const uint16_t* H, long total, int32_t S, const OT* T, int nent, OT* out, u64* zero_counts, hipStream_t st) {
+template <typename HT, typename OT>
+static int launch_score_s1_from_hist_t(const HT* H, long total, int32_t S, const OT* T, int nent, OT* out, u64* zero_counts, hipStream_t st) {
+    constexpr bool PACKED = sizeof(HT) == 4;
     const size_t tbytes = (size_t)nent * sizeof(OT);
+    const long units = total / 4;
     const int rev = 1;
     if (tbytes <= 150 * 1024) {
         const int per_cu = tbytes <= 75 * 1024 ? 2 : 1;
-        long nb = (total / 4 + 4095) / 4096;
+        long nb = (units + 4095) / 4096;
         if (nb > (long)num_cus() * per_cu) nb = (long)num_cus() * per_cu;
         if (nb < 1) nb = 1;
-        auto kern = k_score_s1_from_hist<OT, true>;
         static DynLds lds_attr;
-        EPG_HIP(ensure_dyn_lds(lds_attr, reinterpret_cast<const void*>(kern), 150 * 1024));
-        hipLaunchKernelGGL(kern, dim3((int)nb), dim3(1024), tbytes, st, H, total, S, T, nent, out, zero_counts, rev);
+        if constexpr (PACKED) {
+            auto kern = k_score_s1_from_packed<OT, true>;
+            EPG_HIP(ensure_dyn_lds(lds_attr, reinterpret_cast<const void*>(kern), 150 * 1024));
+            hipLaunchKernelGGL(kern, dim3((int)nb), dim3(1024), tbytes, st, H, total, S, T, nent, out, zero_counts, rev);
+        } else {
+            auto kern = k_score_s1_from_hist<OT, true>;
+            EPG_HIP(ensure_dyn_lds(lds_attr, reinterpret_cast<const void*>(kern), 150 * 1024));
+            hipLaunchKernelGGL(kern, dim3((int)nb), dim3(1024), tbytes, st, H, total, S, T, nent, out, zero_counts, rev);
+        }
     } else {
-        long nb = (total / 4 + 1023) / 1024;
+        long nb = (units + 1023) / 1024;
         if (nb > num_cus() * 8L) nb = num_cus() * 8L;
         if (nb < 1) nb = 1;
-        hipLaunchKernelGGL((k_score_s1_from_hist<OT, false>), dim3((int)nb), dim3(256), 0, st, H, total, S, T, nent, out, zero_counts, rev);
-    }
-    EPG_LAUNCH_CHECK("k_score_s1_from_hist");
+        if constexpr (PACKED) hipLaunchKernelGGL((k_score_s1_from_packed<OT, false>), dim3((int)nb), dim3(256), 0, st, H, total, S, T, nent, out, zero_counts, rev);
+        else hipLaunchKernelGGL((k_score_s1_from_hist<OT, false>), dim3((int)nb), dim3(256), 0, st, H, total, S, T, nent, out, zero_counts, rev);
+    }
+    EPG_LAUNCH_CHECK(PACKED ? "k_score_s1_from_packed" : "k_score_s1_from_hist");
     return EPG_OK;
 }
 
-static int launch_score_s1_from_hist(const uint16_t* H, int64_t R, int32_t N, int32_t S, const double* T64, const float* T32,
+template <typename HT>
+static int launch_score_s1_from_hist(const HT* H, int64_t R, int32_t N, int32_t S, const double* T64, const float* T32,
                                      double* out64, float* out32, hipStream_t st, u64* zero_counts = nullptr) {
     const long total = (long)R * S;
     const int nent = (N + 1) * S;
     int rc = EPG_OK;
-    if (out32) rc = launch_score_s1_from_hist_t<float>(H, total, S, T32, nent, out32, zero_counts, st);
-    if (!rc && out64) rc = launch_score_s1_from_hist_t<double>(H, total, S, T64, nent, out64, out32 ? nullptr : zero_counts, st);
+    if (out32) rc = launch_score_s1_from_hist_t<HT, float>(H, total, S, T32, nent, out32, zero_counts, st);
+    if (!rc && out64) rc = launch_score_s1_from_hist_t<HT, double>(H, total, S, T64, nent, out64, out32 ? nullptr : zero_counts, st);
     return rc;
 }
 
@@ -556,16 +721,32 @@
     return launch_score_s1_from_hist(H, R, N, S, T64, T32, out64, out32, st);
 }
 
-extern "C" int epg_score_s1_from_binhist_table(const uint16_t* H, int64_t R, int32_t N, int32_t S, const double* T64, const float* T32,
-                                               double* out64, float* out32, void* stream) {
+template <typename HT>
+static int score_s1_from_table_impl(const HT* H, int64_t R, int32_t N, int32_t S, const double* T64, const float* T32, double* out64, float* out32,
+                                    void* stream) {
+    constexpr bool PACKED = sizeof(HT) == 4;
     if (R < 0 || N < 1 || S < 1) return fail(EPG_ERR_INVALID_ARG, "score_s1: bad shape");
+    if (PACKED) {
+        const int rc = check_packed("score_s1_from_packed_table", 1, S);
+        if (rc) return rc;
+    }
     if (R == 0) return EPG_OK;
     if (!H || (out64 && !T64) || (out32 && !T32)) return fail(EPG_ERR_INVALID_ARG, "score_s1_from_binhist_table: NULL argument");
     if ((T64 && (reinterpret_cast<uintptr_t>(T64) & 7)) || (T32 && (reinterpret_cast<uintptr_t>(T32) & 3)))
         return fail(EPG_ERR_INVALID_ARG, "score_s1_from_binhist_table: misaligned table");
-    int rc = check_score_from_hist_args(H, out64, out32);
+    int rc = check_score_from_hist_args(H, out64, out32, PACKED ? 16 : 8);
     if (rc) return rc;
     return launch_score_s1_from_hist(H, R, N, S, T64, T32, out64, out32, (hipStream_t)stream);
+}
+
+extern "C" int epg_score_s1_from_binhist_table(const uint16_t* H, int64_t R, int32_t N, int32_t S, const double* T64, const float* T32,
+                                               double* out64, float* out32, void* stream) {
+    return score_s1_from_table_impl(H, R, N, S, T64, T32, out64, out32, stream);
+}
+
+extern "C" int epgs_score_s1_from_packed_table(const uint32_t* P, int64_t R, int32_t N, int32_t S, const double* T64, const float* T32,
+                                               double* out64, float* out32, void* stream) {
+    return score_s1_from_table_impl(P, R, N, S, T64, T32, out64, out32, stream);
 }
 
 __global__ __launch_bounds__(256) void k_s1_combine(const u64* __restrict__ counts, int N, int S, float* __restrict__ q,
@@ -592,14 +773,20 @@
     }
 }
 
-extern "C" int epg_combine_score_s1(int64_t* counts, int32_t rezero, const uint16_t* H, int64_t R, int32_t N, int32_t S, float* q,
-                                    double* out64, float* out32, void* ws, int64_t ws_bytes, void* stream) {
+template <typename HT>
+static int combine_score_s1_impl(int64_t* counts, int32_t rezero, const HT* H, int64_t R, int32_t N, int32_t S, float* q, double* out64, float* out32,
+                                 void* ws, int64_t ws_bytes, void* stream) {
+    constexpr bool PACKED = sizeof(HT) == 4;
     hipStream_t st = (hipStream_t)stream;
     if (R < 0 || N < 1 || S < 1) return fail(EPG_ERR_INVALID_ARG, "combine_score_s1: bad shape R=%lld N=%d S=%d", (long long)R, N, S);
     if (S > 127) return fail(EPG_ERR_UNSUPPORTED, "combine_score_s1: S=%d > 127 (states are int8)", S);
+    if (PACKED) {
+        const int rc = check_packed("combine_score_s1_packed", 1, S);
+        if (rc) return rc;
+    }
     if (!counts || !q || !ws || (R > 0 && !H)) return fail(EPG_ERR_INVALID_ARG, "combine_score_s1: NULL argument");
     if (ws_bytes < s1_table_bytes(N, S)) return fail(EPG_ERR_WORKSPACE, "combine_score_s1: workspace %lld < %lld bytes", (long long)ws_bytes, (long long)s1_table_bytes(N, S));
-    int rc = check_score_from_hist_args(H, out64, out32);
+    int rc = check_score_from_hist_args(H, out64, out32, PACKED ? 16 : 8);
     if (rc) return rc;
     double* T64 = reinterpret_cast<double*>(ws);
     float* T32 = reinterpret_cast<float*>(reinterpret_cast<char*>(ws) + align_up((int64_t)(N + 1) * S * 8, 256));
@@ -611,6 +798,16 @@
         return EPG_OK;
     }
     return launch_score_s1_from_hist(H, R, N, S, T64, T32, out64, out32, st, rezero ? reinterpret_cast<u64*>(counts) : nullptr);
+}
+
+extern "C" int epg_combine_score_s1(int64_t* counts, int32_t rezero, const uint16_t* H, int64_t R, int32_t N, int32_t S, float* q,
+                                    double* out64, float* out32, void* ws, int64_t ws_bytes, void* stream) {
+    return combine_score_s1_impl(counts, rezero, H, R, N, S, q, out64, out32, ws, ws_bytes, stream);
+}
+
+extern "C" int epgs_combine_score_s1_packed(int64_t* counts, int32_t rezero, const uint32_t* P, int64_t R, int32_t N, int32_t S, float* q,
+                                            double* out64, float* out32, void* ws, int64_t ws_bytes, void* stream) {
+    return combine_score_s1_impl(counts, rezero, P, R, N, S, q, out64, out32, ws, ws_bytes, stream);
 }
 
 extern "C" int epg_hist_s1(const int8_t* X, int64_t R, int32_t N, int64_t ldx, int32_t S, int64_t* counts, void* stream) {
diff --git a/epilogos_amd/engine.py b/epilogos_amd/engine.py
--- a/epilogos_amd/engine.py
+++ b/epilogos_amd/engine.py
@@ -111,18 +111,28 @@
     st["stream"] = cur
 
 
-def alloc_hist(X, N, S):
+def packed_ok(N, S):
+    return S % 3 == 0 and 0 < S <= 30 and 0 < N <= 1023
+
+
+def _hist_view(flat_bytes, R, S, row_bytes):
+    t = flat_bytes[:R * row_bytes]
+    return t.view(torch.int16).view(R, S) if row_bytes == 2 * S else t.view(torch.int32).view(R, row_bytes // 4)
+
+
+def alloc_hist(X, N, S, row_bytes=None):
     import os
     R = X.shape[0]
     dev = X.device
     hbytes = R * S * 2
-    plain = lambda: torch.empty((R, S), dtype=torch.int16, device=dev)
+    row_bytes = 2 * S if row_bytes is None else row_bytes
+    plain = lambda: _hist_view(torch.empty(R * row_bytes, dtype=torch.int8, device=dev), R, S, row_bytes)
     if X.numel() < PLACE_MIN_BYTES or not placement_enabled():
         return plain()
     st = _placement.get(dev.index)
     stor = X.untyped_storage()
     key = (stor.data_ptr(), stor.nbytes())
-    view = lambda home: home[:hbytes].view(torch.int16).view(R, S)
+    view = lambda home: _hist_view(home, R, S, row_bytes)
     eager = os.environ.get("EPILOGOS_PLACEMENT_EAGER") == "1"
     if st is not None and st["home"] is not None and st["home"].numel() >= hbytes:
         users = _storage_users(st["home"])
@@ -166,7 +176,7 @@
     st.update(home=home, report=report, stream=torch.cuda.current_stream(), tier=want)
     if home is None and eager and want == 1:
         return alloc_hist(X, N, S)
-    return view(home) if home is not None else h_plain
+    return view(home) if home is not None else _hist_view(h_plain.view(torch.int8).view(-1), R, S, row_bytes)
 
 
 PLACE_SLOW_ALLOC_MS = 20.0
@@ -297,6 +307,19 @@
     return H, counts
 
 
+def bin_hist_packed(X, N, S, counts=None, P=None):
+    R, ldx = _check_states(X, N)
+    if P is None:
+        P = torch.empty((R, S // 3), dtype=torch.int32, device=X.device)
+    _abi.call("epgs_bin_hist_packed", _ptr(X), R, N, ldx, S, _ptr(P), _ptr(counts), _stream())
+    return P, counts
+
+
+def unpack_hist(P, S):
+    p = P.to(torch.int64) & 0xffffffff
+    return torch.stack([(p >> (10 * t)) & 0x3ff for t in range(3)], dim=-1).reshape(P.shape[0], -1)[:, :S].to(torch.int16)
+
+
 def bin_hist_s2(X, N, S, counts2=None, H=None, counts=None):
     R, ldx = _check_states(X, N)
     if H is None:
@@ -311,11 +334,13 @@
     return (C.c_void_p * len(ts))(*[t.data_ptr() if t is not None and t.numel() else None for t in ts])
 
 
-def hist_rows_flat(rows, S, device, dtype=torch.int16):
+def hist_rows_flat(rows, S, device, dtype=torch.int16, row_bytes=None):
     starts, at = [], 0
     for r in rows:
         starts.append(at)
         at += (r + 7) // 8 * 8
+    if row_bytes is not None and row_bytes != 2 * S:
+        return torch.empty((max(at, 1), row_bytes // 4), dtype=torch.int32, device=device), starts
     return torch.empty((max(at, 1), S), dtype=dtype, device=device), starts
 
 
@@ -332,7 +357,8 @@
     dev = Xs[0].device
     if Hs is None and want_hist:
         Hs = hist_rows_alloc([r for r, _l in shapes], S, dev)
-    _abi.call("epg_bin_hist_parts", n, _ptr_array(Xs), (C.c_int64 * n)(*[r for r, _l in shapes]), (C.c_int32 * n)(*[int(N or 1) for N in Ns]),
+    packed = Hs is not None and any(H is not None and H.dtype == torch.int32 for H in Hs)
+    _abi.call("epgs_bin_hist_parts_packed" if packed else "epg_bin_hist_parts", n, _ptr_array(Xs), (C.c_int64 * n)(*[r for r, _l in shapes]), (C.c_int32 * n)(*[int(N or 1) for N in Ns]),
               (C.c_int64 * n)(*[l for _r, l in shapes]), S, _ptr_array(Hs) if Hs is not None else None, _ptr(counts), _stream())
     return Hs, counts
 
@@ -449,7 +475,7 @@
         if T is not None and (T.dtype != dt or T.numel() != (N + 1) * S or not T.is_contiguous()):
             raise ValueError("S1 table must be a contiguous [N + 1, S] tensor of its output's dtype")
     o32, o64 = _outs(R, S, H.device, T32 is not None, T64 is not None, out32, out64)
-    _abi.call("epg_score_s1_from_binhist_table", _ptr(H), R, N, S, _ptr(T64), _ptr(T32), _ptr(o64), _ptr(o32), _stream())
+    _abi.call("epgs_score_s1_from_packed_table" if H.dtype == torch.int32 else "epg_score_s1_from_binhist_table", _ptr(H), R, N, S, _ptr(T64), _ptr(T32), _ptr(o64), _ptr(o32), _stream())
     return o32, o64
 
 
@@ -460,8 +486,8 @@
         q = torch.empty(S, dtype=torch.float32, device=H.device)
     if ws is None:
         ws = _ws(1, 0, N, S, H.device)
-    _abi.call("epg_combine_score_s1", _ptr(counts), 1 if rezero else 0, _ptr(H), R, N, S, _ptr(q), _ptr(o64), _ptr(o32),
-              _ptr(ws), ws.numel(), _stream())
+    _abi.call("epgs_combine_score_s1_packed" if H.dtype == torch.int32 else "epg_combine_score_s1", _ptr(counts), 1 if rezero else 0, _ptr(H),
+              R, N, S, _ptr(q), _ptr(o64), _ptr(o32), _ptr(ws), ws.numel(), _stream())
     return q, o32, o64
 
 
```

After: 5708. 1.7% lower.
